# amathislab/myochallenge

Measured on AMD Instinct MI355X. Metric: env-steps/sec (Baoding, 4096 envs), higher is better.
Workload: dtype f64

## Files before the change

### include/myobatch.h

```cpp
#ifndef MYOBATCH_H
#define MYOBATCH_H

#include <stddef.h>
#include <stdint.h>

#ifdef __cplusplus
extern "C" {
#endif

#define MYO_OK 0
#define MYO_E_ARG -1
#define MYO_E_BADARG MYO_E_ARG
#define MYO_E_UNSUPPORTED -2
#define MYO_E_DEVICE -3
#define MYO_E_STATE -4

typedef struct myo_model myo_model;
typedef struct myo_batch myo_batch;

enum { MYO_F64 = 0, MYO_MIXED = 1, MYO_F32 = 1 };
enum { MYO_TASK_NONE = 0, MYO_TASK_BAODING_P1 = 1, MYO_TASK_BAODING_P2 = 2, MYO_TASK_REORIENT = 3, MYO_TASK_POSE = 4 };
enum { MYO_POSE_RESET_INIT = 0, MYO_POSE_RESET_RANDOM = 1, MYO_POSE_RESET_SDS = 2 };
enum { MYO_POSE_TARGET_GENERATE = 0, MYO_POSE_TARGET_FIXED = 1 };
enum { MYO_WHICH_HOLD = 0, MYO_WHICH_CW = 1, MYO_WHICH_CCW = 2 };
// ... 192 lines not shown
int myo_rollout_policy_input(const float* obs, int N, int O, float* obs_buf, uint16_t* x_bf16, int copies,
                             const int32_t* t_idx, void* stream);
int myo_rollout_sample(const uint16_t* mean_bf16, const uint16_t* value_bf16, const float* log_std, int N, int A,
                       uint64_t seed, uint64_t* draw_counter, const int32_t* t_idx, float* act_buf, float* val_buf,
                       float* logp_buf, float* clipped, int deterministic, void* stream);
int myo_vecnorm_step(const float* obs, const float* rew, const uint8_t* done, const uint8_t* trunc, const float* term_obs,
                     int N, int O, double* obs_mean, double* obs_var, double* obs_count, double* ret_stats,
                     double* returns, double gamma, double eps, double clip_obs, double clip_rew, int training,
                     int norm_obs, int norm_reward, float* nobs, float* starts, const int32_t* t_idx, float* rew_buf,
                     float* start_buf, float* term_buf, float* trunc_buf, double* work, void* stream);
int myo_rollout_sample_sde(const float* mean, const float* latent, const float* exploration_mat, const float* log_std, int N, int L,
                           int A, float* actions, float* clipped, float* logp, int deterministic, void* stream);

int myo_vecnorm_batch_moments(const float* obs, const float* rew, int N, int O, double* returns, double gamma, int training,
                              double* work, double* batch, void* stream);
int myo_vecnorm_finish(const float* obs, const float* rew, const uint8_t* done, const uint8_t* trunc, const float* term_obs,
                       int N, int O, double* obs_mean, double* obs_var, double* obs_count, double* ret_stats, double* returns,
                       double eps, double clip_obs, double clip_rew, int training, int norm_obs, int norm_reward, float* nobs,
                       float* starts, const int32_t* t_idx, float* rew_buf, float* start_buf, float* term_buf, float* trunc_buf,
                       const double* batch, void* stream);
int myo_rollout_advance(int32_t* t_idx, int T, uint64_t* draw_counter, void* stream);
int myo_rollout_state_snapshot(const void* h, const float* c32, int G, int N, int H, const int32_t* t_idx, int seq_len, int S,
                               void* h_snap, float* c_snap, void* stream);

int myo_lstm_cell_fwd(const void* gx, const void* gh, const void* c_prev, const float* keep_next, int R, int N, int H,
                      int is_bf16, void* out_h, void* hm_next, void* cm_next, void* c_new, void* ws, void* stream);
int myo_lstm_cell_bwd(const void* dout, const void* dhm_next, const void* dcm_next, const float* keep_next,
                      const void* c_prev, const void* c_new, const void* ws, int R, int N, int H, int is_bf16,
                      void* dgates, void* dc_prev, void* stream);

int myo_lstm_step_supported(int H);
int myo_lstm_step_fwd(const void* gx, long long gx_sg, long long gx_sr, const void* h_prev, const void* c_prev, const void* w_hh,
                      const float* keep_next, int G, int N, int H, void* out_h, long long out_sg, void* hm_next, void* cm_next,
                      void* c_new, void* ws, const float* c_prev32, float* cm_next32, void* stream);
int myo_lstm_step_bwd(const void* dout, long long dout_sg, const void* dgates_next, const void* dcm_next, const void* w_hh_t,
                      const float* keep_next, const void* c_prev, const void* c_new, const void* ws, int G, int N, int H,
                      void* dgates, void* dc_prev, void* stream);

int myo_lstm_seq_supported(int H);
int myo_lstm_seq_fwd(const void* gx, long long gx_st, long long gx_sg, long long gx_sr, void* hm, void* cm, const void* w_frag,
                     const float* keep, int G, int N, int H, int T, int row_split, void* out_h, long long out_sg, long long out_st,
                     void* c_new, void* ws, const float* c0_32, void* stream);
int myo_lstm_seq_bwd(const void* dout, long long dout_sg, long long dout_st, const void* wt_frag, const float* keep, const void* cm,
                     const void* c_new, const void* ws, int G, int N, int H, int T, int row_split, void* dgates, void* stream);

int myo_gae(const float* rew, const float* val, const float* starts, const float* last_val,
            const float* last_done, int T, int N, float gamma, float lam, float* adv, float* ret,
            void* stream);

#define MYO_HP_LR 0
#define MYO_HP_CLIP 1
#define MYO_HP_KL_LIMIT 2
#define MYO_HP_STOP 3
#define MYO_HP_APPLIED 4
#define MYO_HP_COUNT 5
#define MYO_HP_SUM_KL 6
#define MYO_HP_SUM_CLIPFRAC 7
#define MYO_HP_SUM_ENTLOSS 8
#define MYO_HP_LAST_KL 9
#define MYO_HP_LAST_PL 10
#define MYO_HP_LAST_VL 11
#define MYO_HP_WORDS 16
typedef struct myo_ppo_mlp_desc {
  const float *obs, *act, *oldlp, *adv, *ret;
  const int64_t* idx;
  int32_t B, O, A, hidden;
  const float* params;
  float* grads;
  int64_t G;
  int64_t off_W1[2], off_b1[2], off_W2[2], off_b2[2], off_Wh[2], off_bh[2], off_log_std;
  float clip, vf_coef, ent_coef;
  int32_t compute_adv_stats;
  float* adv_stats;
  float* acc;
  void* workspace;
  int64_t workspace_bytes;
  float* sqnorm_part;
  int32_t* adam_step;
  float* hp;
} myo_ppo_mlp_desc;
int myo_ppo_mlp_sqnorm_parts(int act_dim);
long long myo_ppo_mlp_workspace_bytes(int B, int obs_dim, int act_dim, int hidden, long long G);
int myo_ppo_mlp_step(const myo_ppo_mlp_desc* d, void* stream);

typedef struct myo_ppo_mlp_rollout_desc {
  const float* obs;
  int32_t N, O, A, hidden;
  const float* params;
  int64_t off_W1[2], off_b1[2], off_W2[2], off_b2[2], off_Wh[2], off_bh[2], off_log_std;
  uint64_t seed;
  uint64_t* draw_counter;
  const int32_t* t_idx;
  float *obs_buf, *act_buf, *val_buf, *logp_buf, *clipped;
  int32_t deterministic;
  void* workspace;
  int64_t workspace_bytes;
} myo_ppo_mlp_rollout_desc;
long long myo_ppo_mlp_rollout_workspace_bytes(int obs_dim, int act_dim, int hidden);
int myo_ppo_mlp_rollout_refresh(const myo_ppo_mlp_rollout_desc* d, void* stream);
int myo_ppo_mlp_rollout(const myo_ppo_mlp_rollout_desc* d, void* stream);

int myo_adam_clip_step(float* p, const float* g, float* m, float* v, int n, float lr, float b1, float b2,
                       float eps, float max_norm, float grad_scale, int* step, float* scratch, uint16_t* p_bf16,
                       void* stream);
int myo_adam_apply(float* p, const float* g, float* m, float* v, int n, float lr, float b1, float b2,
                   float eps, float max_norm, float grad_scale, const int* step, const float* scratch, int nparts,
                   uint16_t* p_bf16, void* stream);
int myo_adam_clip_step_hp(float* p, const float* g, float* m, float* v, int n, float lr, float b1, float b2,
                          float eps, float max_norm, float grad_scale, int* step, float* scratch, uint16_t* p_bf16,
                          float* hp, void* stream);
int myo_adam_apply_hp(float* p, const float* g, float* m, float* v, int n, float lr, float b1, float b2,
                      float eps, float max_norm, float grad_scale, const int* step, const float* scratch, int nparts,
                      uint16_t* p_bf16, float* hp, void* stream);

const char* myo_last_error(void);
const char* myo_version(void);

#ifdef __cplusplus
}
#endif
#endif
```

### myochallenge_amd/csrc/myo_ppo_mlp.h

```cpp
#pragma once
#ifndef MYO_EMU

typedef __attribute__((ext_vector_type(8))) __bf16 myo_bf16x8;
typedef __attribute__((ext_vector_type(4))) float myo_f32x4;

#define MLP_H 256
#define MLP_OPMAX 128
#define MLP_APM 48
#define MLP_AKP 64
#define MLP_XS (MLP_OPMAX + 8)
#define MLP_HS (MLP_H + 8)
#define MLP_DS (MLP_AKP + 8)
#define MLP_SOS 49
#define MLP_SPLITK 16

struct MlpArgs {
  const float *obs, *act, *oldlp, *adv, *ret;
  const long long* idx;
  const float *log_std, *adv_stats;
  const unsigned short *W1p, *W2, *W2T, *Whp, *WhT;
  const float* bias;
  unsigned short *XT, *H1T, *H2T, *dH1T, *dH2T, *dOT;
  float* part;
  int B, O, A, OP, NB;
  float clip, vf_coef;
  const float* hp;
};

__device__ __forceinline__ unsigned short mlp_f2bf(float x) {
  unsigned u = __float_as_uint(x);
  u += 0x7fffu + ((u >> 16) & 1u);
  return (unsigned short)(u >> 16);
}
__device__ __forceinline__ float mlp_bf2f(unsigned short h) { return __uint_as_float((unsigned)h << 16); }

struct MlpPrepArgs {
  const float* p;
  long long off_W1[2], off_b1[2], off_W2[2], off_b2[2], off_Wh[2], off_bh[2];
  int O, OP, Ah[2];
  unsigned short *W1p, *W2, *W2T, *Whp, *WhT;
  float* bias;
  const float* adv_part;
  float* adv_stats;
  int adv_nb, B;
};

#define MLP_ADV_BLOCKS 64
__global__ void __launch_bounds__(256) k_mlp_prep(MlpPrepArgs P) {
  if (P.adv_nb > 0 && blockIdx.x == gridDim.x - 1) {
    __shared__ float sp[3 * MLP_ADV_BLOCKS];
    const int t = threadIdx.x;
    if (t < 3 * P.adv_nb) sp[t] = P.adv_part[t];
    __syncthreads();
    if (t == 0) {
      float cn = 0.f, cm = 0.f, c2 = 0.f;
      for (int b = 0; b < P.adv_nb; ++b) {
        const float bn = sp[3 * b], bm = sp[3 * b + 1], b2 = sp[3 * b + 2];
        if (bn > 0.f) {
          const float tot = cn + bn, dl = bm - cm;
          cm += dl * (bn / tot);
          c2 += b2 + dl * dl * (cn * bn / tot);
          cn = tot;
        }
      }
      P.adv_stats[0] = cm; P.adv_stats[1] = sqrtf(c2 / (P.B > 1 ? P.B - 1 : 1));
    }
  }
  constexpr int H = MLP_H;
  const long long tid = (long long)blockIdx.x * blockDim.x + threadIdx.x, nth = (long long)gridDim.x * blockDim.x;
  for (int net = 0; net < 2; ++net) {
    const float* W1 = P.p + P.off_W1[net]; const float* W2 = P.p + P.off_W2[net]; const float* Wh = P.p + P.off_Wh[net];
    for (long long e = tid; e < (long long)H * P.OP; e += nth) {
      const int o = (int)(e / P.OP), i = (int)(e % P.OP);
      P.W1p[(size_t)net * H * P.OP + e] = i < P.O ? mlp_f2bf(W1[(size_t)o * P.O + i]) : (unsigned short)0;
    }
    for (long long e = tid; e < (long long)H * H; e += nth) {
      const int o = (int)(e / H), i = (int)(e % H);
      const unsigned short v = mlp_f2bf(W2[e]);
      P.W2[(size_t)net * H * H + e] = v;
      P.W2T[(size_t)net * H * H + (size_t)i * H + o] = v;
    }
    for (long long e = tid; e < (long long)MLP_APM * H; e += nth) {
      const int a = (int)(e / H), h = (int)(e % H);
      P.Whp[(size_t)net * MLP_APM * H + e] = a < P.Ah[net] ? mlp_f2bf(Wh[(size_t)a * H + h]) : (unsigned short)0;
    }
    for (long long e = tid; e < (long long)H * MLP_AKP; e += nth) {
      const int h = (int)(e / MLP_AKP), a = (int)(e % MLP_AKP);
      P.WhT[(size_t)net * H * MLP_AKP + e] = a < P.Ah[net] ? mlp_f2bf(Wh[(size_t)a * H + h]) : (unsigned short)0;
    }
    for (long long e = tid; e < H; e += nth) {
      P.bias[net * H + e] = P.p[P.off_b1[net] + e];
      P.bias[2 * H + net * H + e] = P.p[P.off_b2[net] + e];
    }
    for (long long e = tid; e < MLP_APM; e += nth) P.bias[4 * H + net * MLP_APM + e] = e < P.Ah[net] ? P.p[P.off_bh[net] + e] : 0.f;
  }
}

__global__ void __launch_bounds__(256) k_adv_moments(const float* __restrict__ adv, const long long* __restrict__ idx, int B,
                                                     float* __restrict__ part) {
  __shared__ float red[4];
  __shared__ float s_mean;
  const int t = threadIdx.x, nb = gridDim.x;
  const int chunk = (B + nb - 1) / nb, lo = blockIdx.x * chunk, hi = min(B, lo + chunk), n = max(hi - lo, 0);
  constexpr int PER = 4;
  float v[PER];
  float s = 0.f;
#pragma unroll
  for (int k = 0; k < PER; ++k) { const int i = lo + t + 256 * k; v[k] = i < hi ? adv[idx[i]] : 0.f; s += v[k]; }
  for (int i = lo + t + 256 * PER; i < hi; i += 256) s += adv[idx[i]];
  for (int off = 32; off >= 1; off >>= 1) s += __shfl_xor(s, off, 64);
  if ((t & 63) == 0) red[t >> 6] = s;
  __syncthreads();
  if (t == 0) s_mean = n ? ((red[0] + red[1]) + (red[2] + red[3])) / n : 0.f;
  __syncthreads();
  const float mean = s_mean;
  float m2 = 0.f;
#pragma unroll
  for (int k = 0; k < PER; ++k) { const float d = v[k] - mean; m2 += (lo + t + 256 * k) < hi ? d * d : 0.f; }
  for (int i = lo + t + 256 * PER; i < hi; i += 256) { const float d = adv[idx[i]] - mean; m2 += d * d; }
  for (int off = 32; off >= 1; off >>= 1) m2 += __shfl_xor(m2, off, 64);
  __syncthreads();
  if ((t & 63) == 0) red[t >> 6] = m2;
  __syncthreads();
  if (t == 0) { part[3 * blockIdx.x] = (float)n; part[3 * blockIdx.x + 1] = mean; part[3 * blockIdx.x + 2] = (red[0] + red[1]) + (red[2] + red[3]); }
}

template <int KSTEPS>
__device__ __forceinline__ void mlp_load_w(myo_bf16x8 (&bw)[8][4], const unsigned short* Wg, int w_stride, int n0, int lm, int lq) {
#pragma unroll
  for (int ks = 0; ks < KSTEPS; ++ks)
#pragma unroll
    for (int nt = 0; nt < 4; ++nt) bw[ks][nt] = *reinterpret_cast<const myo_bf16x8*>(Wg + (size_t)(n0 + 16 * nt + lm) * w_stride + 32 * ks + 8 * lq);
  __builtin_amdgcn_sched_barrier(0);
}
template <int KSTEPS, int MT>
__device__ __forceinline__ void mlp_mma_slab(myo_f32x4 (&acc)[MT][4], const unsigned short* As, int as_stride, const myo_bf16x8 (&bw)[8][4],
                                             int lm, int lq) {
#pragma unroll
  for (int mt = 0; mt < MT; ++mt)
#pragma unroll
    for (int nt = 0; nt < 4; ++nt) acc[mt][nt] = myo_f32x4{0.f, 0.f, 0.f, 0.f};
#pragma unroll
  for (int ks = 0; ks < KSTEPS; ++ks) {
#pragma unroll
    for (int m2 = 0; m2 < MT; m2 += 2) {
      myo_bf16x8 a[2];
#pragma unroll
      for (int mt = 0; mt < 2; ++mt) a[mt] = *reinterpret_cast<const myo_bf16x8*>(As + (16 * (m2 + mt) + lm) * as_stride + 32 * ks + 8 * lq);
#pragma unroll
      for (int mt = 0; mt < 2; ++mt)
#pragma unroll
        for (int nt = 0; nt < 4; ++nt) acc[m2 + mt][nt] = __builtin_amdgcn_mfma_f32_16x16x32_bf16(a[mt], bw[ks][nt], acc[m2 + mt][nt], 0, 0, 0);
    }
  }
  __builtin_amdgcn_sched_barrier(0);
}

#ifdef MLP_PROF
__device__ unsigned long long g_mlp_prof[16];
#define MLP_STAMP(k) { __syncthreads(); if (threadIdx.x == 0 && blockIdx.x == 3 && blockIdx.y == 0) g_mlp_prof[k] = wall_clock64(); }
extern "C" int myo_debug_mlp_prof(unsigned long long* out) { return (int)hipMemcpyFromSymbol(out, HIP_SYMBOL(g_mlp_prof), sizeof g_mlp_prof); }
#else
#define MLP_STAMP(k)
#endif

#ifndef MLP_BM
#define MLP_BM 32
#endif
#define MLP_FWDBWD_LDS (512 + MLP_BM * MLP_XS * 2 + MLP_BM * MLP_HS * 2 + MLP_BM * MLP_SOS * 4 + MLP_BM * MLP_DS * 2 + 128 * 4 + 192 * 4)

template <int MT>
__device__ __forceinline__ unsigned long long mlp_store_act(const myo_f32x4 (&acc)[MT][4], const float (&bb)[4], unsigned short* Hs, unsigned short* HT,
                                                            size_t B, int r0, int n0, int lm, int lq) {
  static_assert(MT * 16 <= 64, "one mask bit per accumulator element");
  unsigned long long mask = 0;
#pragma unroll
  for (int mt = 0; mt < MT; ++mt)
#pragma unroll
    for (int nt = 0; nt < 4; ++nt) {
      const int n = n0 + 16 * nt + lm, m = 16 * mt + 4 * lq;
      unsigned short h[4];
#pragma unroll
      for (int r = 0; r < 4; ++r) {
        h[r] = mlp_f2bf(fmaxf(acc[mt][nt][r] + bb[nt], 0.f)); Hs[(m + r) * MLP_HS + n] = h[r];
        mask |= (unsigned long long)(h[r] != 0) << (16 * mt + 4 * nt + r);
      }
      *reinterpret_cast<uint2*>(HT + (size_t)n * B + r0 + m) = make_uint2((unsigned)h[0] | ((unsigned)h[1] << 16), (unsigned)h[2] | ((unsigned)h[3] << 16));
    }
  return mask;
}
template <int MT, bool TO_LDS>
__device__ __forceinline__ void mlp_store_grad(const myo_f32x4 (&acc)[MT][4], unsigned long long mask, unsigned short* Hs, unsigned short* HT, size_t B,
                                               int r0, int n0, int lm, int lq) {
#pragma unroll
  for (int mt = 0; mt < MT; ++mt)
#pragma unroll
    for (int nt = 0; nt < 4; ++nt) {
      const int n = n0 + 16 * nt + lm, m = 16 * mt + 4 * lq;
      unsigned short h[4];
#pragma unroll
      for (int r = 0; r < 4; ++r) {
        const unsigned short on = (unsigned short)(-(int)((mask >> (16 * mt + 4 * nt + r)) & 1ull));
        h[r] = mlp_f2bf(acc[mt][nt][r]) & on;
        if (TO_LDS) Hs[(m + r) * MLP_HS + n] = h[r];
      }
      *reinterpret_cast<uint2*>(HT + (size_t)n * B + r0 + m) = make_uint2((unsigned)h[0] | ((unsigned)h[1] << 16), (unsigned)h[2] | ((unsigned)h[3] << 16));
    }
}

__global__ void __launch_bounds__(256, 2) k_mlp_fwdbwd(MlpArgs P) {
  constexpr int H = MLP_H, XS = MLP_XS, HS = MLP_HS, DS = MLP_DS, SOS = MLP_SOS, BM = MLP_BM, MT = BM / 16, RW = BM / 4;
  extern __shared__ __align__(16) unsigned char mlp_smem[];
  long long* s_idx = reinterpret_cast<long long*>(mlp_smem);
  unsigned short* Xs = reinterpret_cast<unsigned short*>(mlp_smem + 512);
  float* So = reinterpret_cast<float*>(mlp_smem + 512);
  unsigned short* Hs = Xs + BM * XS;
  float* Sa = reinterpret_cast<float*>(Hs + BM * HS);
  unsigned short* dOs = reinterpret_cast<unsigned short*>(Sa + BM * SOS);
  float* s_ls = reinterpret_cast<float*>(dOs + BM * DS);
  float* s_row = s_ls + 128;
  static_assert(BM * MLP_SOS * 4 <= BM * MLP_XS * 2, "the head output tile fits where X was");
  static_assert(BM == 32 || BM == 64, "wave / tile mapping below");
  const int t = threadIdx.x, w = t >> 6, lane = t & 63, lm = lane & 15, lq = lane >> 4;
  const int net = blockIdx.y, blk = blockIdx.x, r0 = blk * BM, B = P.B, O = P.O, A = P.A, OP = P.OP;
  const int n0 = 64 * w;
  MLP_STAMP(0)
  if (t < BM) s_idx[t] = P.idx[r0 + t];
  if (t < A) { const float ls = P.log_std[t]; s_ls[t] = ls; s_ls[64 + t] = __expf(-ls); }
  const float* b1 = P.bias + net * H; const float* b2 = P.bias + 2 * H + net * H; const float* bh = P.bias + 4 * H + net * MLP_APM;
  float bb1[4], bb2[4];
#pragma unroll
  for (int nt = 0; nt < 4; ++nt) { bb1[nt] = b1[n0 + 16 * nt + lm]; bb2[nt] = b2[n0 + 16 * nt + lm]; }
  myo_bf16x8 bw[8][4];
  {
    const unsigned short* W1 = P.W1p + (size_t)net * H * OP;
    if (OP == 96) mlp_load_w<3>(bw, W1, OP, n0, lm, lq);
    else if (OP == 128) mlp_load_w<4>(bw, W1, OP, n0, lm, lq);
    else if (OP == 64) mlp_load_w<2>(bw, W1, OP, n0, lm, lq);
    else mlp_load_w<1>(bw, W1, OP, n0, lm, lq);
  }
  __syncthreads();
  if (t < BM) {
    const size_t src = (size_t)s_idx[t];
// ... 303 lines not shown

__global__ void __launch_bounds__(256) k_mlp_wgrad(MlpWgradArgs P) {
  const int jid = blockIdx.x % P.njobs, split = blockIdx.x / P.njobs;
  const MlpWgradJob J = P.job[jid];
  const int t = threadIdx.x, w = t >> 6, lane = t & 63, lm = lane & 15, lq = lane >> 4;
  const int wm = w >> 1, wn = w & 1, B = P.B;
  const int mb = J.m0 + 64 * wm, nb = J.n0 + 64 * wn;
  const size_t k0 = (size_t)split * P.rows_per_split;
  myo_f32x4 acc[4][4], accb[4];
#pragma unroll
  for (int mt = 0; mt < 4; ++mt) {
    accb[mt] = myo_f32x4{0.f, 0.f, 0.f, 0.f};
#pragma unroll
    for (int nt = 0; nt < 4; ++nt) acc[mt][nt] = myo_f32x4{0.f, 0.f, 0.f, 0.f};
  }
  const bool do_bias = J.bias_off >= 0 && nb == 0;
  myo_bf16x8 ones;
#pragma unroll
  for (int j = 0; j < 8; ++j) ones[j] = (__bf16)1.0f;
  const int ksteps = P.rows_per_split / 32;
  const unsigned short* ap[4]; const unsigned short* bp[4];
#pragma unroll
  for (int q = 0; q < 4; ++q) { ap[q] = J.AT + (size_t)(mb + 16 * q + lm) * B + k0 + 8 * lq; bp[q] = J.BT + (size_t)(nb + 16 * q + lm) * B + k0 + 8 * lq; }
  myo_bf16x8 a0[4], b0[4], a1[4], b1[4];
#pragma unroll
  for (int q = 0; q < 4; ++q) { a0[q] = *reinterpret_cast<const myo_bf16x8*>(ap[q]); b0[q] = *reinterpret_cast<const myo_bf16x8*>(bp[q]); }
  for (int ks = 0; ks < ksteps; ks += 2) {
#pragma unroll
    for (int q = 0; q < 4; ++q) { a1[q] = *reinterpret_cast<const myo_bf16x8*>(ap[q] + 32 * (ks + 1)); b1[q] = *reinterpret_cast<const myo_bf16x8*>(bp[q] + 32 * (ks + 1)); }
#pragma unroll
    for (int mt = 0; mt < 4; ++mt)
#pragma unroll
      for (int nt = 0; nt < 4; ++nt) acc[mt][nt] = __builtin_amdgcn_mfma_f32_16x16x32_bf16(a0[mt], b0[nt], acc[mt][nt], 0, 0, 0);
    if (do_bias) {
#pragma unroll
      for (int mt = 0; mt < 4; ++mt) accb[mt] = __builtin_amdgcn_mfma_f32_16x16x32_bf16(a0[mt], ones, accb[mt], 0, 0, 0);
    }
    if (ks + 2 < ksteps) {
#pragma unroll
      for (int q = 0; q < 4; ++q) { a0[q] = *reinterpret_cast<const myo_bf16x8*>(ap[q] + 32 * (ks + 2)); b0[q] = *reinterpret_cast<const myo_bf16x8*>(bp[q] + 32 * (ks + 2)); }
    }
#pragma unroll
    for (int mt = 0; mt < 4; ++mt)
#pragma unroll
      for (int nt = 0; nt < 4; ++nt) acc[mt][nt] = __builtin_amdgcn_mfma_f32_16x16x32_bf16(a1[mt], b1[nt], acc[mt][nt], 0, 0, 0);
    if (do_bias) {
#pragma unroll
      for (int mt = 0; mt < 4; ++mt) accb[mt] = __builtin_amdgcn_mfma_f32_16x16x32_bf16(a1[mt], ones, accb[mt], 0, 0, 0);
    }
  }
  float* out = P.slab + (size_t)split * P.G;
#pragma unroll
  for (int mt = 0; mt < 4; ++mt)
#pragma unroll
    for (int nt = 0; nt < 4; ++nt)
#pragma unroll
      for (int r = 0; r < 4; ++r) {
        const int m = mb + 16 * mt + 4 * lq + r, n = nb + 16 * nt + lm;
        if (m < J.M && n < J.N) out[J.out_off + (size_t)m * J.ldo + n] = acc[mt][nt][r];
      }
  if (do_bias && lm == 0) {
#pragma unroll
    for (int mt = 0; mt < 4; ++mt)
#pragma unroll
      for (int r = 0; r < 4; ++r) {
        const int m = mb + 16 * mt + 4 * lq + r;
        if (m < J.M) out[J.bias_off + m] = accb[mt][r];
      }
  }
}

#define MLP_RF_BLOCKS 256
struct MlpRfArgs {
  const float* slab; float* g; long long G; int splits;
  const float* part; float* acc; int NB, A; float ent_coef;
  long long off_log_std, off_bh0, off_bh1;
  float* sq_part; int* adam_step;
  float* hp;
};
__global__ void __launch_bounds__(256) k_mlp_reduce_finish(MlpRfArgs P) {
  __shared__ float red[4];
  const int t = threadIdx.x, A = P.A;
  if ((int)blockIdx.x < MLP_RF_BLOCKS) {
    float sq = 0.f;
    for (long long e = (long long)blockIdx.x * 256 + t; e < P.G; e += (long long)MLP_RF_BLOCKS * 256) {
      float s = 0.f;
#pragma unroll 4
      for (int k = 0; k < P.splits; ++k) s += P.slab[(size_t)k * P.G + e];
      const bool theirs = (e >= P.off_log_std && e < P.off_log_std + A) || (e >= P.off_bh0 && e < P.off_bh0 + A) || e == P.off_bh1;
      if (!theirs) { P.g[e] = s; sq += s * s; }
    }
    for (int off = 32; off >= 1; off >>= 1) sq += __shfl_xor(sq, off, 64);
    if ((t & 63) == 0) red[t >> 6] = sq;
    float pl = 0.f, vl = 0.f, kl = 0.f, cf = 0.f, el = 0.f;
    if (P.hp && blockIdx.x == 0 && t < 64) {
      pl = myo_col_sum(P.part, A, P.NB, t); vl = myo_col_sum(P.part, A + 1, P.NB, t);
      kl = myo_col_sum(P.part, 2 * A + 3, P.NB, t); cf = myo_col_sum(P.part, 2 * A + 4, P.NB, t); el = myo_col_sum(P.part, 2 * A + 5, P.NB, t);
    }
    __syncthreads();
    if (t == 0) {
      P.sq_part[blockIdx.x] = (red[0] + red[1]) + (red[2] + red[3]);
      if (blockIdx.x == 0) {
        const bool stopped = P.hp ? myo_hp_record(P.hp, pl, vl, kl, cf, el) : false;
        if (!stopped) { const int done = P.adam_step[1]; P.adam_step[0] = done; P.adam_step[1] = done + 1; }
      }
    }
    return;
  }
  const int c = (int)blockIdx.x - MLP_RF_BLOCKS;
  if (t >= 64) return;
  float a = 0.f;
  for (int b = t; b < P.NB; b += 64) a += P.part[(size_t)c * P.NB + b];
  for (int off = 32; off >= 1; off >>= 1) a += __shfl_xor(a, off, 64);
  if (t == 0) {
    P.acc[c] = a;
    float w = 0.f;
    if (c < A) { w = a - P.ent_coef; P.g[P.off_log_std + c] = w; }
    else if (c >= A + 2 && c < 2 * A + 2) { w = a; P.g[P.off_bh0 + c - A - 2] = w; }
    else if (c == 2 * A + 2) { w = a; P.g[P.off_bh1] = w; }
    P.sq_part[MLP_RF_BLOCKS + c] = w * w;
  }
}

__global__ void __launch_bounds__(256) k_mlp_reduce(const float* __restrict__ slab, float* __restrict__ g, long long G, int splits) {
  const long long e = (long long)blockIdx.x * 256 + threadIdx.x;
  if (e >= G) return;
  float s = 0.f;
#pragma unroll 4
  for (int k = 0; k < splits; ++k) s += slab[(size_t)k * G + e];
  g[e] = s;
}
#endif
```

### myochallenge_amd/csrc/myobatch.hip

```cpp
#include <hip/hip_runtime.h>
#include <utility>
#include <vector>
#define MYO_BACKEND_NAME "gfx950"
#define MYO_BACKEND_DENSE_NEWTON 0
#define MYO_BACKEND_BATCH_FIELDS hipEvent_t ev0, ev1; std::vector<std::pair<hipEvent_t, hipEvent_t>> pending;
#define MYO_BACKEND_RENDER_ENVS_MAX 65535
struct DeviceGuard {
  int prev = -1; bool switched = false;
  explicit DeviceGuard(int dev) { if (hipGetDevice(&prev) == hipSuccess && prev != dev) switched = (hipSetDevice(dev) == hipSuccess); }
  ~DeviceGuard() { if (switched) (void)hipSetDevice(prev); }
};
#include "myo_host.h"

static int be_malloc(void** p, size_t n) { return (int)hipMalloc(p, n ? n : 1); }
static void be_free(void* p) { (void)hipFree(p); }
static int be_h2d(void* d, const void* h, size_t n) { return (int)hipMemcpy(d, h, n, hipMemcpyHostToDevice); }
static int be_set_device(int dev) { return (int)hipSetDevice(dev); }
static const char* be_errstr(int e) { return hipGetErrorString((hipError_t)e); }

#define MYO_MAX_DEVICES 64
struct BoundDev { const myo_batch* b = nullptr; hipStream_t last = nullptr; bool have_last = false; hipEvent_t ev = nullptr; };
static BoundDev g_bound[MYO_MAX_DEVICES];
static std::mutex g_bound_mu;
struct SlotWs { double* p = nullptr; int* map = nullptr; int users = 0; char* big = nullptr; int big_users = 0; };
// ... 531 lines not shown
                                                 const float* __restrict__ log_std, const float* __restrict__ adv_stats,
                                                 int B, int A, float clip, float vf_coef, float* __restrict__ dmean,
                                                 float* __restrict__ dvalue, float* __restrict__ acc,
                                                 unsigned short* __restrict__ dmean_h, unsigned short* __restrict__ dvalue_h,
                                                 float* __restrict__ part, const float* __restrict__ hp) {
  __shared__ float t_mean[64 * 64], t_act[64 * 64], s_ls[64], s_inv[64];
  if (hp) clip = hp[MYO_HP_CLIP];
  const int lane = threadIdx.x, r0 = blockIdx.x * 64;
  const int rows = (B - r0) < 64 ? (B - r0) : 64;
  const int n = rows * A;
  const size_t base = (size_t)r0 * A;
  const unsigned short* mean_h = reinterpret_cast<const unsigned short*>(mean);
  for (int k = lane; k < n; k += 64) {
    t_mean[k] = IN_BF16 ? __uint_as_float(((unsigned)mean_h[base + k]) << 16) : mean[base + k];
    t_act[k] = actions[base + k];
  }
  if (lane < A) { const float ls = log_std[lane]; s_ls[lane] = ls; s_inv[lane] = __expf(-ls); }
  __syncthreads();
  const int i = r0 + lane;
  const bool on = lane < rows;
  float pl_i = 0.f, vl_i = 0.f, dlogp = 0.f, dv_i = 0.f, kl_i = 0.f, cf_i = 0.f, el_i = 0.f;
  if (on) {
    float logp = 0.f, ent = 0.f;
    for (int a = 0; a < A; ++a) {
      const float z = (t_act[lane * A + a] - t_mean[lane * A + a]) * s_inv[a];
      logp += -0.5f * z * z - s_ls[a] - 0.9189385332046727f;
      ent += s_ls[a] + 1.4189385332046727f;
    }
    const float an = (adv[i] - adv_stats[0]) / (adv_stats[1] + 1e-8f);
    const float lr_i = logp - old_logp[i];
    const float ratio = __expf(lr_i);
    kl_i = ((ratio - 1.f) - lr_i) / B;
    cf_i = (fabsf(ratio - 1.f) > clip ? 1.f : 0.f) / B;
    el_i = -ent / B;
    const float s1 = an * ratio;
    const float rc = fminf(fmaxf(ratio, 1.f - clip), 1.f + clip);
    const float s2 = an * rc;
    pl_i = -fminf(s1, s2) / B;
    const bool inside = (ratio > 1.f - clip) && (ratio < 1.f + clip);
    dlogp = -(an * ratio) * ((s1 <= s2) ? 1.f : (inside ? 1.f : 0.f)) / B;
    const float val = IN_BF16 ? __uint_as_float(((unsigned)reinterpret_cast<const unsigned short*>(values)[i]) << 16) : values[i];
    const float dv = val - returns[i];
    vl_i = dv * dv / B;
    dv_i = vf_coef * 2.f / B * dv;
    dvalue[i] = dv_i;
    if (dvalue_h) dvalue_h[i] = myo_f2bf(dv_i);
  }
  if (on) {
    for (int a = 0; a < A; ++a) {
      const float inv = s_inv[a];
      const float z = (t_act[lane * A + a] - t_mean[lane * A + a]) * inv;
      t_mean[lane * A + a] = dlogp * z * inv;
      t_act[lane * A + a] = dlogp * (z * z - 1.f);
    }
  }
  __syncthreads();
  float my_ls = 0.f, my_db = 0.f;
  if (lane < A)
    for (int r = 0; r < rows; ++r) { my_ls += t_act[r * A + lane]; my_db += t_mean[r * A + lane]; }
  for (int k = lane; k < n; k += 64) {
    const float v = t_mean[k];
    dmean[base + k] = v;
    if (dmean_h) dmean_h[base + k] = myo_f2bf(v);
  }
  for (int off = 32; off >= 1; off >>= 1) {
    pl_i += __shfl_xor(pl_i, off, 64); vl_i += __shfl_xor(vl_i, off, 64); dv_i += __shfl_xor(dv_i, off, 64);
  }
  const int W = 2 * A + 3, NB = gridDim.x;
  if (lane < A) { part[(size_t)lane * NB + blockIdx.x] = my_ls; part[(size_t)(A + 2 + lane) * NB + blockIdx.x] = my_db; }
  if (lane == 0) {
    part[(size_t)A * NB + blockIdx.x] = pl_i; part[(size_t)(A + 1) * NB + blockIdx.x] = vl_i;
    part[(size_t)(2 * A + 2) * NB + blockIdx.x] = dv_i;
  }
  if (hp) {
    for (int off = 32; off >= 1; off >>= 1) {
      kl_i += __shfl_xor(kl_i, off, 64); cf_i += __shfl_xor(cf_i, off, 64); el_i += __shfl_xor(el_i, off, 64);
    }
    if (lane == 0) {
      part[(size_t)W * NB + blockIdx.x] = kl_i; part[(size_t)(W + 1) * NB + blockIdx.x] = cf_i;
      part[(size_t)(W + 2) * NB + blockIdx.x] = el_i;
    }
  }
}
__device__ __forceinline__ bool myo_hp_record(float* __restrict__ hp, float pl, float vl, float kl, float cf, float el) {
  int* hi = reinterpret_cast<int*>(hp);
  if (hi[MYO_HP_STOP]) return true;
  hp[MYO_HP_SUM_KL] += kl; hp[MYO_HP_SUM_CLIPFRAC] += cf; hp[MYO_HP_SUM_ENTLOSS] += el;
  hi[MYO_HP_COUNT] += 1;
  hp[MYO_HP_LAST_KL] = kl; hp[MYO_HP_LAST_PL] = pl; hp[MYO_HP_LAST_VL] = vl;
  const float lim = hp[MYO_HP_KL_LIMIT];
  if (lim > 0.f && kl > lim) { hi[MYO_HP_STOP] = 1; return true; }
  return false;
}
__device__ __forceinline__ float myo_col_sum(const float* __restrict__ part, int c, int NB, int lane) {
  float a = 0.f;
  for (int b = lane; b < NB; b += 64) a += part[(size_t)c * NB + b];
  for (int off = 32; off >= 1; off >>= 1) a += __shfl_xor(a, off, 64);
  return a;
}
__global__ void __launch_bounds__(64) k_colmajor_finish(const float* __restrict__ part, float* __restrict__ acc, int NB, int A,
                                                        float ent_coef, float* __restrict__ g_log_std,
                                                        float* __restrict__ g_bias_pi, float* __restrict__ g_bias_vf,
                                                        float* __restrict__ hp) {
  const int c = blockIdx.x, lane = threadIdx.x;
  if (c == 2 * A + 3) {
    const float pl = myo_col_sum(part, A, NB, lane), vl = myo_col_sum(part, A + 1, NB, lane);
    const float kl = myo_col_sum(part, c, NB, lane), cf = myo_col_sum(part, c + 1, NB, lane), el = myo_col_sum(part, c + 2, NB, lane);
    if (lane == 0) (void)myo_hp_record(hp, pl, vl, kl, cf, el);
    return;
  }
  float a = 0.f;
  for (int b = lane; b < NB; b += 64) a += part[(size_t)c * NB + b];
  for (int off = 32; off >= 1; off >>= 1) a += __shfl_xor(a, off, 64);
  if (lane == 0) {
    acc[c] = a;
    if (g_log_std && c < A) g_log_std[c] = a - ent_coef;
    if (g_bias_pi && c >= A + 2 && c < 2 * A + 2) g_bias_pi[c - A - 2] = a;
    if (g_bias_vf && c == 2 * A + 2) g_bias_vf[0] = a;
  }
}
static int ppo_loss_grad(const float* mean, const float* values, const float* actions, const float* old_logp,
                         const float* adv, const float* returns, const float* log_std, const float* adv_stats,
                         int B, int A, float clip, float vf_coef, float* dmean, float* dvalue, float* acc,
                         uint16_t* dmean_bf16, uint16_t* dvalue_bf16, float* work, int in_bf16, float ent_coef,
                         float* g_log_std, float* g_bias_pi, float* g_bias_vf, float* hp, void* stream) {
  if (!mean || !values || !actions || !old_logp || !adv || !returns || !log_std || !adv_stats || !dmean || !dvalue || !acc ||
      !work || B <= 0 || A <= 0 || A > 64)
    return fail(MYO_E_ARG, "myo_ppo_loss_grad: bad arguments");
  hipStream_t st = (hipStream_t)stream;
  const int nblk = (B + 63) / 64;
  if (in_bf16)
    hipLaunchKernelGGL(k_ppo_loss<true>, dim3(nblk), dim3(64), 0, st, mean, values, actions, old_logp, adv, returns,
                       log_std, adv_stats, B, A, clip, vf_coef, dmean, dvalue, acc, dmean_bf16, dvalue_bf16, work, (const float*)hp);
  else
    hipLaunchKernelGGL(k_ppo_loss<false>, dim3(nblk), dim3(64), 0, st, mean, values, actions, old_logp, adv, returns,
                       log_std, adv_stats, B, A, clip, vf_coef, dmean, dvalue, acc, dmean_bf16, dvalue_bf16, work, (const float*)hp);
  hipLaunchKernelGGL(k_colmajor_finish, dim3(2 * A + 3 + (hp ? 1 : 0)), dim3(64), 0, st, work, acc, nblk, A, ent_coef, g_log_std, g_bias_pi,
                     g_bias_vf, hp);
  LAUNCH_CHECK(0)
  return MYO_OK;
}
extern "C" int myo_ppo_loss_grad(const float* mean, const float* values, const float* actions, const float* old_logp,
                                 const float* adv, const float* returns, const float* log_std, const float* adv_stats,
                                 int B, int A, float clip, float vf_coef, float* dmean, float* dvalue, float* acc,
                                 uint16_t* dmean_bf16, uint16_t* dvalue_bf16, float* work, int in_bf16, float ent_coef,
                                 float* g_log_std, float* g_bias_pi, float* g_bias_vf, void* stream) {
  return ppo_loss_grad(mean, values, actions, old_logp, adv, returns, log_std, adv_stats, B, A, clip, vf_coef, dmean, dvalue, acc,
                       dmean_bf16, dvalue_bf16, work, in_bf16, ent_coef, g_log_std, g_bias_pi, g_bias_vf, nullptr, stream);
}
extern "C" int myo_ppo_loss_grad_hp(const float* mean, const float* values, const float* actions, const float* old_logp,
                                    const float* adv, const float* returns, const float* log_std, const float* adv_stats,
                                    int B, int A, float clip, float vf_coef, float* dmean, float* dvalue, float* acc,
                                    uint16_t* dmean_bf16, uint16_t* dvalue_bf16, float* work, int in_bf16, float ent_coef,
                                    float* g_log_std, float* g_bias_pi, float* g_bias_vf, float* hp, void* stream) {
  return ppo_loss_grad(mean, values, actions, old_logp, adv, returns, log_std, adv_stats, B, A, clip, vf_coef, dmean, dvalue, acc,
                       dmean_bf16, dvalue_bf16, work, in_bf16, ent_coef, g_log_std, g_bias_pi, g_bias_vf, hp, stream);
}

template <bool BF16>
__global__ void __launch_bounds__(256) k_splitk_reduce(const unsigned* __restrict__ part, float2* __restrict__ out, int splits,
                                                       int n2, int total2) {
  const int j = blockIdx.x * blockDim.x + threadIdx.x;
  if (j >= total2) return;
  const int g = j / n2, c = j - g * n2;
  float a0 = 0.f, a1 = 0.f;
  if (BF16) {
    const unsigned* src = part + (size_t)g * splits * n2 + c;
#pragma unroll 8
    for (int k = 0; k < splits; ++k) {
      const unsigned u = src[(size_t)k * n2];
      a0 += __uint_as_float(u << 16);
      a1 += __uint_as_float(u & 0xffff0000u);
    }
  } else {
    const float2* src = reinterpret_cast<const float2*>(part) + (size_t)g * splits * n2 + c;
// ... 702 lines not shown
}
template <typename E>
__global__ void __launch_bounds__(256) k_lstm_cell_bwd(const E* __restrict__ dout, const E* __restrict__ dhm_next, const E* __restrict__ dcm_next,
                                                       const float* __restrict__ keep_next, const E* __restrict__ c_prev,
                                                       const E* __restrict__ c_new, const E* __restrict__ ws, int R, int N, int H,
                                                       E* __restrict__ dgates, E* __restrict__ dc_prev) {
  const size_t idx = (size_t)blockIdx.x * blockDim.x + threadIdx.x;
  if (idx >= (size_t)R * H) return;
  const int r = (int)(idx / H), j = (int)(idx % H);
  const size_t g0 = (size_t)r * 4 * H + j;
  const float k = keep_next ? keep_next[r % N] : 1.f;
  const float dh = (dout ? myo_ld(dout, idx) : 0.f) + (dhm_next ? k * myo_ld(dhm_next, idx) : 0.f);
  const float dc_in = dcm_next ? k * myo_ld(dcm_next, idx) : 0.f;
  const float i = myo_ld(ws, g0), f = myo_ld(ws, g0 + H), g = myo_ld(ws, g0 + 2 * H), o = myo_ld(ws, g0 + 3 * H);
  const float tc = tanhf(myo_ld(c_new, idx));
  const float dct = dc_in + dh * o * (1.f - tc * tc);
  myo_st(dgates, g0, dct * g * i * (1.f - i));
  myo_st(dgates, g0 + H, dct * myo_ld(c_prev, idx) * f * (1.f - f));
  myo_st(dgates, g0 + 2 * H, dct * i * (1.f - g * g));
  myo_st(dgates, g0 + 3 * H, dh * tc * o * (1.f - o));
  myo_st(dc_prev, idx, dct * f);
}
extern "C" int myo_lstm_cell_fwd(const void* gx, const void* gh, const void* c_prev, const float* keep_next, int R, int N, int H,
                                 int is_bf16, void* out_h, void* hm_next, void* cm_next, void* c_new, void* ws, void* stream) {
  if (!gx || !gh || !c_prev || !out_h || !hm_next || !cm_next || !c_new || !ws || R <= 0 || N <= 0 || H <= 0 || R % N)
    return fail(MYO_E_ARG, "myo_lstm_cell_fwd: bad arguments");
  const unsigned nb = (unsigned)(((size_t)R * H + 255) / 256);
  if (is_bf16)
    hipLaunchKernelGGL(k_lstm_cell_fwd<unsigned short>, dim3(nb), dim3(256), 0, (hipStream_t)stream, (const unsigned short*)gx,
                       (const unsigned short*)gh, (const unsigned short*)c_prev, keep_next, R, N, H, (unsigned short*)out_h,
                       (unsigned short*)hm_next, (unsigned short*)cm_next, (unsigned short*)c_new, (unsigned short*)ws);
  else
    hipLaunchKernelGGL(k_lstm_cell_fwd<float>, dim3(nb), dim3(256), 0, (hipStream_t)stream, (const float*)gx, (const float*)gh,
                       (const float*)c_prev, keep_next, R, N, H, (float*)out_h, (float*)hm_next, (float*)cm_next, (float*)c_new,
                       (float*)ws);
  LAUNCH_CHECK(0)
  return MYO_OK;
}
extern "C" int myo_lstm_cell_bwd(const void* dout, const void* dhm_next, const void* dcm_next, const float* keep_next,
                                 const void* c_prev, const void* c_new, const void* ws, int R, int N, int H, int is_bf16,
                                 void* dgates, void* dc_prev, void* stream) {
  if (!c_prev || !c_new || !ws || !dgates || !dc_prev || R <= 0 || N <= 0 || H <= 0 || R % N)
    return fail(MYO_E_ARG, "myo_lstm_cell_bwd: bad arguments");
  const unsigned nb = (unsigned)(((size_t)R * H + 255) / 256);
  if (is_bf16)
    hipLaunchKernelGGL(k_lstm_cell_bwd<unsigned short>, dim3(nb), dim3(256), 0, (hipStream_t)stream, (const unsigned short*)dout,
                       (const unsigned short*)dhm_next, (const unsigned short*)dcm_next, keep_next, (const unsigned short*)c_prev,
                       (const unsigned short*)c_new, (const unsigned short*)ws, R, N, H, (unsigned short*)dgates,
                       (unsigned short*)dc_prev);
  else
    hipLaunchKernelGGL(k_lstm_cell_bwd<float>, dim3(nb), dim3(256), 0, (hipStream_t)stream, (const float*)dout, (const float*)dhm_next,
                       (const float*)dcm_next, keep_next, (const float*)c_prev, (const float*)c_new, (const float*)ws, R, N, H,
                       (float*)dgates, (float*)dc_prev);
  LAUNCH_CHECK(0)
  return MYO_OK;
}

__global__ void k_gae(const float* __restrict__ rew, const float* __restrict__ val, const float* __restrict__ starts,
                      const float* __restrict__ last_val, const float* __restrict__ last_done, int T, int N, float gamma,
                      float lam, float* __restrict__ adv, float* __restrict__ ret) {
  const int e = blockIdx.x * blockDim.x + threadIdx.x;
  if (e >= N) return;
  float last = 0.f, nextv = last_val[e], nonterm = 1.f - last_done[e];
  for (int t = T - 1; t >= 0; --t) {
    const size_t i = (size_t)t * N + e;
    const float v = val[i];
    const float delta = rew[i] + gamma * nextv * nonterm - v;
    last = delta + gamma * lam * nonterm * last;
    adv[i] = last;
    ret[i] = last + v;
    nextv = v;
    nonterm = 1.f - starts[i];
  }
}
extern "C" int myo_gae(const float* rew, const float* val, const float* starts, const float* last_val, const float* last_done,
                       int T, int N, float gamma, float lam, float* adv, float* ret, void* stream) {
  if (!rew || !val || !starts || !last_val || !last_done || !adv || !ret || T <= 0 || N <= 0) return fail(MYO_E_ARG, "myo_gae: bad arguments");
  hipLaunchKernelGGL(k_gae, dim3((N + 255) / 256), dim3(256), 0, (hipStream_t)stream, rew, val, starts, last_val, last_done, T, N,
                     gamma, lam, adv, ret);
  LAUNCH_CHECK(0)
  return MYO_OK;
}

#define MYO_SQN_BLOCKS 64
__global__ void __launch_bounds__(256) k_grad_sqnorm(const float* __restrict__ g, int n, float gs, float* __restrict__ part,
                                                     int* __restrict__ step, const float* __restrict__ hp) {
  float acc = 0.f;
  for (int i = blockIdx.x * 256 + threadIdx.x; i < n; i += MYO_SQN_BLOCKS * 256) { const float x = g[i] * gs; acc += x * x; }
  for (int off = 32; off >= 1; off >>= 1) acc += __shfl_xor(acc, off, 64);
  __shared__ float red[4];
  if ((threadIdx.x & 63) == 0) red[threadIdx.x >> 6] = acc;
  __syncthreads();
  if (threadIdx.x == 0) {
    part[blockIdx.x] = (red[0] + red[1]) + (red[2] + red[3]);
    if (blockIdx.x == 0 && !(hp && reinterpret_cast<const int*>(hp)[MYO_HP_STOP])) { const int done = step[1]; step[0] = done; step[1] = done + 1; }
  }
}
__global__ void __launch_bounds__(256) k_adam(float* __restrict__ p, const float* __restrict__ g, float* __restrict__ m,
                                              float* __restrict__ v, int n, float lr, float b1, float b2, float eps,
                                              float max_norm, float gs, const int* __restrict__ step,
                                              const float* __restrict__ part, unsigned short* __restrict__ p_bf16, int nparts,
                                              float* __restrict__ hp) {
  if (hp) {
    if (reinterpret_cast<const int*>(hp)[MYO_HP_STOP]) return;
    lr = hp[MYO_HP_LR];
  }
  __shared__ float sq_red[256];
  {
    float a = 0.f;
    for (int k = threadIdx.x; k < nparts; k += 256) a += part[k];
    sq_red[threadIdx.x] = a;
    __syncthreads();
    for (int w = 128; w >= 1; w >>= 1) { if ((int)threadIdx.x < w) sq_red[threadIdx.x] += sq_red[threadIdx.x + w]; __syncthreads(); }
  }
  const float sq = sq_red[0];
  const int t = step[1];
  const float norm = sqrtf(sq);
  const float clip = (max_norm > 0.f) ? fminf(1.f, max_norm / (norm + 1e-6f)) : 1.f;
  const float bc1 = 1.f - powf(b1, (float)t), bc2 = 1.f - powf(b2, (float)t);
  const float step_size = lr / bc1, inv_sqrt_bc2 = rsqrtf(bc2);
  for (int i = blockIdx.x * blockDim.x + threadIdx.x; i < n; i += gridDim.x * blockDim.x) {
    const float gi = g[i] * gs * clip;
    const float mi = b1 * m[i] + (1.f - b1) * gi;
    const float vi = b2 * v[i] + (1.f - b2) * gi * gi;
    m[i] = mi; v[i] = vi;
    const float pn = p[i] - step_size * mi / (sqrtf(vi) * inv_sqrt_bc2 + eps);
    p[i] = pn;
    if (p_bf16) p_bf16[i] = myo_f2bf(pn);
  }
  if (hp && blockIdx.x == 0 && threadIdx.x == 0) reinterpret_cast<int*>(hp)[MYO_HP_APPLIED] += 1;
}
static int adam_clip_step(float* p, const float* g, float* m, float* v, int n, float lr, float b1, float b2,
                          float eps, float max_norm, float grad_scale, int* step, float* scratch, uint16_t* p_bf16,
                          float* hp, void* stream) {
  if (!p || !g || !m || !v || !step || !scratch || n <= 0) return fail(MYO_E_ARG, "myo_adam_clip_step: bad arguments");
  hipStream_t st = (hipStream_t)stream;
  const int blocks = (n + 255) / 256 < 1024 ? (n + 255) / 256 : 1024;
  hipLaunchKernelGGL(k_grad_sqnorm, dim3(MYO_SQN_BLOCKS), dim3(256), 0, st, g, n, grad_scale, scratch, step, (const float*)hp);
  hipLaunchKernelGGL(k_adam, dim3(blocks), dim3(256), 0, st, p, g, m, v, n, lr, b1, b2, eps, max_norm, grad_scale, step, scratch,
                     (unsigned short*)p_bf16, MYO_SQN_BLOCKS, hp);
  LAUNCH_CHECK(0)
  return MYO_OK;
}
extern "C" int myo_adam_clip_step(float* p, const float* g, float* m, float* v, int n, float lr, float b1, float b2,
                                  float eps, float max_norm, float grad_scale, int* step, float* scratch, uint16_t* p_bf16,
                                  void* stream) {
  return adam_clip_step(p, g, m, v, n, lr, b1, b2, eps, max_norm, grad_scale, step, scratch, p_bf16, nullptr, stream);
}
extern "C" int myo_adam_clip_step_hp(float* p, const float* g, float* m, float* v, int n, float lr, float b1, float b2,
                                     float eps, float max_norm, float grad_scale, int* step, float* scratch, uint16_t* p_bf16,
                                     float* hp, void* stream) {
  return adam_clip_step(p, g, m, v, n, lr, b1, b2, eps, max_norm, grad_scale, step, scratch, p_bf16, hp, stream);
}
static int adam_apply(float* p, const float* g, float* m, float* v, int n, float lr, float b1, float b2,
                      float eps, float max_norm, float grad_scale, const int* step, const float* scratch, int nparts,
                      uint16_t* p_bf16, float* hp, void* stream) {
  if (!p || !g || !m || !v || !step || !scratch || n <= 0 || nparts <= 0) return fail(MYO_E_ARG, "myo_adam_apply: bad arguments");
  const int blocks = (n + 255) / 256 < 1024 ? (n + 255) / 256 : 1024;
  hipLaunchKernelGGL(k_adam, dim3(blocks), dim3(256), 0, (hipStream_t)stream, p, g, m, v, n, lr, b1, b2, eps, max_norm, grad_scale, step, scratch,
                     (unsigned short*)p_bf16, nparts, hp);
  LAUNCH_CHECK(0)
  return MYO_OK;
}
extern "C" int myo_adam_apply(float* p, const float* g, float* m, float* v, int n, float lr, float b1, float b2,
                              float eps, float max_norm, float grad_scale, const int* step, const float* scratch, int nparts,
                              uint16_t* p_bf16, void* stream) {
  return adam_apply(p, g, m, v, n, lr, b1, b2, eps, max_norm, grad_scale, step, scratch, nparts, p_bf16, nullptr, stream);
}
extern "C" int myo_adam_apply_hp(float* p, const float* g, float* m, float* v, int n, float lr, float b1, float b2,
                                 float eps, float max_norm, float grad_scale, const int* step, const float* scratch, int nparts,
                                 uint16_t* p_bf16, float* hp, void* stream) {
  return adam_apply(p, g, m, v, n, lr, b1, b2, eps, max_norm, grad_scale, step, scratch, nparts, p_bf16, hp, stream);
}

#include "myo_ppo_mlp.h"
struct MlpWs { unsigned short *W1p, *W2, *W2T, *Whp, *WhT; float* bias; unsigned short *XT, *H1T, *H2T, *dH1T, *dH2T, *dOT; float *part, *slab, *advpart; size_t bytes; };
static MlpWs mlp_carve(unsigned char* base, int B, int OP, int A, long long G) {
  MlpWs w;
  size_t o = 0;
  auto take = [&](size_t n) { unsigned char* p = base ? base + o : nullptr; o += (n + 255) / 256 * 256; return p; };
  const size_t H = MLP_H;
  w.W1p = (unsigned short*)take(2 * H * OP * 2); w.W2 = (unsigned short*)take(2 * H * H * 2); w.W2T = (unsigned short*)take(2 * H * H * 2);
  w.Whp = (unsigned short*)take(2 * MLP_APM * H * 2); w.WhT = (unsigned short*)take(2 * H * MLP_AKP * 2);
  w.bias = (float*)take((4 * H + 2 * MLP_APM) * 4);
  w.XT = (unsigned short*)take((size_t)128 * B * 2);
  w.H1T = (unsigned short*)take(2 * H * (size_t)B * 2); w.H2T = (unsigned short*)take(2 * H * (size_t)B * 2);
  w.dH1T = (unsigned short*)take(2 * H * (size_t)B * 2); w.dH2T = (unsigned short*)take(2 * H * (size_t)B * 2);
  w.dOT = (unsigned short*)take((size_t)256 * B * 2);
  w.part = (float*)take((size_t)(2 * A + 6) * (B / MLP_BM) * 4);
  w.slab = (float*)take((size_t)MLP_SPLITK * G * 4);
  w.advpart = (float*)take(3 * MLP_ADV_BLOCKS * 4);
  w.bytes = o;
  return w;
}
static int mlp_shape_ok(int B, int O, int A, int hidden) {
  return hidden == MLP_H && O >= 1 && O <= MLP_OPMAX && A >= 1 && A <= MLP_APM && B >= 64 * MLP_SPLITK && B % (64 * MLP_SPLITK) == 0;
}
extern "C" long long myo_ppo_mlp_workspace_bytes(int B, int obs_dim, int act_dim, int hidden, long long G) {
  if (!mlp_shape_ok(B, obs_dim, act_dim, hidden) || G <= 0) return -1;
  return (long long)mlp_carve(nullptr, B, (obs_dim + 31) / 32 * 32, act_dim, G).bytes;
}
extern "C" int myo_ppo_mlp_sqnorm_parts(int act_dim) {
  return MLP_RF_BLOCKS + 2 * act_dim + 3;
}
extern "C" int myo_ppo_mlp_step(const myo_ppo_mlp_desc* d, void* stream) {
  if (!d || !d->obs || !d->act || !d->oldlp || !d->adv || !d->ret || !d->idx || !d->params || !d->grads || !d->adv_stats || !d->acc ||
      !d->workspace)
    return fail(MYO_E_ARG, "myo_ppo_mlp_step: null argument");
  const int B = d->B, O = d->O, A = d->A, OP = (O + 31) / 32 * 32;
  if (!mlp_shape_ok(B, O, A, d->hidden)) return fail(MYO_E_UNSUPPORTED, "myo_ppo_mlp_step: needs hidden = %d, obs <= %d, act <= %d, batch a multiple of %d", MLP_H, MLP_OPMAX, MLP_APM, 64 * MLP_SPLITK);
  const MlpWs w = mlp_carve((unsigned char*)d->workspace, B, OP, A, d->G);
  if ((long long)w.bytes > d->workspace_bytes) return fail(MYO_E_ARG, "myo_ppo_mlp_step: workspace too small (%zu bytes needed)", w.bytes);
  hipStream_t st = (hipStream_t)stream;
  static bool lds_set = false;
  if (!lds_set) {
    if (hipFuncSetAttribute((const void*)k_mlp_fwdbwd, hipFuncAttributeMaxDynamicSharedMemorySize, MLP_FWDBWD_LDS) != hipSuccess)
      return fail(MYO_E_DEVICE, "myo_ppo_mlp_step: cannot reserve %d bytes of LDS", (int)MLP_FWDBWD_LDS);
    lds_set = true;
  }
  if (d->compute_adv_stats) hipLaunchKernelGGL(k_adv_moments, dim3(MLP_ADV_BLOCKS), dim3(256), 0, st, d->adv, (const long long*)d->idx, B, w.advpart);
  MlpPrepArgs pp;
  pp.p = d->params; pp.O = O; pp.OP = OP; pp.Ah[0] = A; pp.Ah[1] = 1;
  for (int k = 0; k < 2; ++k) {
    pp.off_W1[k] = d->off_W1[k]; pp.off_b1[k] = d->off_b1[k]; pp.off_W2[k] = d->off_W2[k]; pp.off_b2[k] = d->off_b2[k];
    pp.off_Wh[k] = d->off_Wh[k]; pp.off_bh[k] = d->off_bh[k];
  }
  pp.adv_part = w.advpart; pp.adv_stats = d->adv_stats; pp.adv_nb = d->compute_adv_stats ? MLP_ADV_BLOCKS : 0; pp.B = B;
  pp.W1p = w.W1p; pp.W2 = w.W2; pp.W2T = w.W2T; pp.Whp = w.Whp; pp.WhT = w.WhT; pp.bias = w.bias;
  hipLaunchKernelGGL(k_mlp_prep, dim3(256), dim3(256), 0, st, pp);
  MlpArgs a;
  a.obs = d->obs; a.act = d->act; a.oldlp = d->oldlp; a.adv = d->adv; a.ret = d->ret; a.idx = (const long long*)d->idx;
  a.log_std = d->params + d->off_log_std; a.adv_stats = d->adv_stats;
  a.W1p = w.W1p; a.W2 = w.W2; a.W2T = w.W2T; a.Whp = w.Whp; a.WhT = w.WhT; a.bias = w.bias;
  a.XT = w.XT; a.H1T = w.H1T; a.H2T = w.H2T; a.dH1T = w.dH1T; a.dH2T = w.dH2T; a.dOT = w.dOT; a.part = w.part;
  a.B = B; a.O = O; a.A = A; a.OP = OP; a.NB = B / MLP_BM; a.clip = d->clip; a.vf_coef = d->vf_coef; a.hp = d->hp;
  hipLaunchKernelGGL(k_mlp_fwdbwd, dim3(B / MLP_BM, 2), dim3(256), MLP_FWDBWD_LDS, st, a);
  MlpWgradArgs g;
  g.njobs = 0; g.B = B; g.rows_per_split = B / MLP_SPLITK; g.G = d->G; g.slab = w.slab;
  const size_t HB = (size_t)MLP_H * B;
  for (int net = 0; net < 2; ++net) {
    for (int m0 = 0; m0 < MLP_H; m0 += 128) {
      for (int n0 = 0; n0 < MLP_H; n0 += 128)
        g.job[g.njobs++] = MlpWgradJob{w.dH2T + net * HB, w.H1T + net * HB, MLP_H, MLP_H, MLP_H, m0, n0, d->off_W2[net], n0 == 0 ? d->off_b2[net] : -1};
      g.job[g.njobs++] = MlpWgradJob{w.dH1T + net * HB, w.XT, MLP_H, O, O, m0, 0, d->off_W1[net], d->off_b1[net]};
    }
    for (int n0 = 0; n0 < MLP_H; n0 += 128)
      g.job[g.njobs++] = MlpWgradJob{w.dOT + (size_t)net * 128 * B, w.H2T + net * HB, net == 0 ? A : 1, MLP_H, MLP_H, 0, n0, d->off_Wh[net], -1};
  }
  hipLaunchKernelGGL(k_mlp_wgrad, dim3(g.njobs * MLP_SPLITK), dim3(256), 0, st, g);
  if (d->sqnorm_part && d->adam_step) {
    MlpRfArgs rf;
    rf.slab = w.slab; rf.g = d->grads; rf.G = d->G; rf.splits = MLP_SPLITK; rf.part = w.part; rf.acc = d->acc; rf.NB = B / MLP_BM; rf.A = A;
    rf.ent_coef = d->ent_coef; rf.off_log_std = d->off_log_std; rf.off_bh0 = d->off_bh[0]; rf.off_bh1 = d->off_bh[1];
    rf.sq_part = d->sqnorm_part; rf.adam_step = d->adam_step; rf.hp = d->hp;
    hipLaunchKernelGGL(k_mlp_reduce_finish, dim3(MLP_RF_BLOCKS + 2 * A + 3), dim3(256), 0, st, rf);
  } else {
    hipLaunchKernelGGL(k_mlp_reduce, dim3((unsigned)((d->G + 255) / 256)), dim3(256), 0, st, (const float*)w.slab, d->grads, d->G, MLP_SPLITK);
    hipLaunchKernelGGL(k_colmajor_finish, dim3(2 * A + 3 + (d->hp ? 1 : 0)), dim3(64), 0, st, (const float*)w.part, d->acc, B / MLP_BM, A, d->ent_coef,
                       d->grads + d->off_log_std, d->grads + d->off_bh[0], d->grads + d->off_bh[1], d->hp);
  }
  LAUNCH_CHECK(0)
  return MYO_OK;
}

struct MlpImg { unsigned short *W1p, *W2, *W2T, *Whp, *WhT; float* bias; size_t bytes; };
static MlpImg mlp_carve_images(unsigned char* base, int OP) {
  MlpImg w;
  size_t o = 0;
  auto take = [&](size_t n) { unsigned char* p = base ? base + o : nullptr; o += (n + 255) / 256 * 256; return p; };
  const size_t H = MLP_H;
  w.W1p = (unsigned short*)take(2 * H * OP * 2); w.W2 = (unsigned short*)take(2 * H * H * 2); w.W2T = (unsigned short*)take(2 * H * H * 2);
  w.Whp = (unsigned short*)take(2 * MLP_APM * H * 2); w.WhT = (unsigned short*)take(2 * H * MLP_AKP * 2);
  w.bias = (float*)take((4 * H + 2 * MLP_APM) * 4);
  w.bytes = o;
  return w;
}
static int mlp_rollout_ok(const myo_ppo_mlp_rollout_desc* d) {
  return d->hidden == MLP_H && d->O >= 1 && d->O <= MLP_OPMAX && d->A >= 1 && d->A <= MLP_APM && d->N >= MLP_BM && d->N % MLP_BM == 0;
}
extern "C" long long myo_ppo_mlp_rollout_workspace_bytes(int obs_dim, int act_dim, int hidden) {
  if (hidden != MLP_H || obs_dim < 1 || obs_dim > MLP_OPMAX || act_dim < 1 || act_dim > MLP_APM) return -1;
  return (long long)mlp_carve_images(nullptr, (obs_dim + 31) / 32 * 32).bytes;
}
extern "C" int myo_ppo_mlp_rollout_refresh(const myo_ppo_mlp_rollout_desc* d, void* stream) {
  if (!d || !d->params || !d->workspace) return fail(MYO_E_ARG, "myo_ppo_mlp_rollout_refresh: null argument");
  if (!mlp_rollout_ok(d)) return fail(MYO_E_UNSUPPORTED, "myo_ppo_mlp_rollout: needs hidden = %d, obs <= %d, act <= %d, envs a multiple of %d", MLP_H, MLP_OPMAX, MLP_APM, MLP_BM);
  const int OP = (d->O + 31) / 32 * 32;
  const MlpImg w = mlp_carve_images((unsigned char*)d->workspace, OP);
  if ((long long)w.bytes > d->workspace_bytes) return fail(MYO_E_ARG, "myo_ppo_mlp_rollout_refresh: workspace too small (%zu bytes needed)", w.bytes);
  MlpPrepArgs pp;
  pp.p = d->params; pp.O = d->O; pp.OP = OP; pp.Ah[0] = d->A; pp.Ah[1] = 1;
  for (int k = 0; k < 2; ++k) {
    pp.off_W1[k] = d->off_W1[k]; pp.off_b1[k] = d->off_b1[k]; pp.off_W2[k] = d->off_W2[k]; pp.off_b2[k] = d->off_b2[k];
    pp.off_Wh[k] = d->off_Wh[k]; pp.off_bh[k] = d->off_bh[k];
  }
  pp.adv_part = nullptr; pp.adv_stats = nullptr; pp.adv_nb = 0; pp.B = 0;
  pp.W1p = w.W1p; pp.W2 = w.W2; pp.W2T = w.W2T; pp.Whp = w.Whp; pp.WhT = w.WhT; pp.bias = w.bias;
  hipLaunchKernelGGL(k_mlp_prep, dim3(256), dim3(256), 0, (hipStream_t)stream, pp);
  LAUNCH_CHECK(0)
  return MYO_OK;
}
extern "C" int myo_ppo_mlp_rollout(const myo_ppo_mlp_rollout_desc* d, void* stream) {
  if (!d || !d->obs || !d->params || !d->draw_counter || !d->t_idx || !d->act_buf || !d->val_buf || !d->logp_buf || !d->clipped || !d->workspace)
    return fail(MYO_E_ARG, "myo_ppo_mlp_rollout: null argument");
  if (!mlp_rollout_ok(d)) return fail(MYO_E_UNSUPPORTED, "myo_ppo_mlp_rollout: needs hidden = %d, obs <= %d, act <= %d, envs a multiple of %d", MLP_H, MLP_OPMAX, MLP_APM, MLP_BM);
  const int OP = (d->O + 31) / 32 * 32;
  const MlpImg w = mlp_carve_images((unsigned char*)d->workspace, OP);
  if ((long long)w.bytes > d->workspace_bytes) return fail(MYO_E_ARG, "myo_ppo_mlp_rollout: workspace too small (%zu bytes needed)", w.bytes);
  MlpPolicyArgs a;
  a.obs = d->obs; a.log_std = d->params + d->off_log_std; a.W1p = w.W1p; a.W2 = w.W2; a.Whp = w.Whp; a.bias = w.bias;
  a.obs_buf = d->obs_buf; a.act_buf = d->act_buf; a.val_buf = d->val_buf; a.logp_buf = d->logp_buf; a.clipped = d->clipped;
  a.t_idx = d->t_idx; a.draw_counter = (unsigned long long*)d->draw_counter; a.seed = d->seed;
  a.N = d->N; a.O = d->O; a.A = d->A; a.OP = OP; a.deterministic = d->deterministic;
  hipLaunchKernelGGL(k_mlp_policy, dim3(d->N / MLP_BM, 2), dim3(256), MLP_POLICY_LDS, (hipStream_t)stream, a);
  LAUNCH_CHECK(0)
  return MYO_OK;
}

#include "myo_lstm_step.h"
extern "C" int myo_lstm_step_supported(int H) { return (H == 32 || H == 64 || H == 128 || H == 256) ? 1 : 0; }
extern "C" int myo_lstm_step_fwd(const void* gx, long long gx_sg, long long gx_sr, const void* h_prev, const void* c_prev, const void* w_hh,
                                 const float* keep_next, int G, int N, int H, void* out_h, long long out_sg, void* hm_next, void* cm_next,
                                 void* c_new, void* ws, const float* c_prev32, float* cm_next32, void* stream) {
  if (!gx || !h_prev || (!c_prev && !c_prev32) || !w_hh || !out_h || !hm_next || (!cm_next && !cm_next32) || G <= 0 || N <= 0 || H <= 0 || (gx_sg & 3) || (gx_sr & 3) || (out_sg & 3))
    return fail(MYO_E_ARG, "myo_lstm_step_fwd: bad arguments");
  if (!myo_lstm_step_supported(H)) return fail(MYO_E_UNSUPPORTED, "myo_lstm_step_fwd: hidden size %d (32, 64, 128 or 256)", H);
  typedef const unsigned short* cu;
  typedef unsigned short* mu;
#define MYO_LSTM_FWD(HH)                                                                                                              \
  lstm_step_fwd_launch<HH>((cu)gx, gx_sg, gx_sr, (cu)h_prev, (cu)c_prev, (cu)w_hh, keep_next, G, N, (mu)out_h, out_sg, (mu)hm_next,   \
                           (mu)cm_next, (mu)c_new, (mu)ws, c_prev32, cm_next32, (hipStream_t)stream)
  switch (H) {
    case 32: MYO_LSTM_FWD(32); break;
    case 64: MYO_LSTM_FWD(64); break;
    case 128: MYO_LSTM_FWD(128); break;
    default: MYO_LSTM_FWD(256); break;
  }
#undef MYO_LSTM_FWD
  LAUNCH_CHECK(0)
  return MYO_OK;
}
extern "C" int myo_lstm_step_bwd(const void* dout, long long dout_sg, const void* dgates_next, const void* dcm_next, const void* w_hh_t,
                                 const float* keep_next, const void* c_prev, const void* c_new, const void* ws, int G, int N, int H,
// ... 55 lines not shown
```

### myochallenge_amd/native.py

```python
from __future__ import annotations

import ctypes as C
import os
from typing import Optional

import numpy as np

_HERE = os.path.dirname(os.path.abspath(__file__))
LIB_PATH = os.path.join(_HERE, "libmyobatch.so")

MYO_F64, MYO_MIXED = 0, 1
MYO_F32 = MYO_MIXED
TASK_NONE, TASK_BAODING_P1, TASK_BAODING_P2, TASK_REORIENT, TASK_POSE = 0, 1, 2, 3, 4
POSE_RESET_INIT, POSE_RESET_RANDOM, POSE_RESET_SDS = 0, 1, 2
POSE_TARGET_GENERATE, POSE_TARGET_FIXED = 0, 1
CHOICE_FIXED, CHOICE_CW, CHOICE_CCW, CHOICE_RANDOM = 0, 1, 2, 3
MUSCLE_NONE, MUSCLE_FATIGUE, MUSCLE_REAFFERENTATION = 0, 1, 2
N_RWD = 8
RWD_KEYS = ("pos_dist_1", "pos_dist_2", "act_reg", "alive", "sparse", "solved", "done", "dense")


ROT_CHOICE_MAX, OBJG_MAX, POSE_NQ_MAX = 4, 20, 38


# ... 114 lines not shown
        vp, i32, u64, dbl = C.c_void_p, C.c_int, C.c_uint64, C.c_double
        L.myo_last_error.restype = C.c_char_p
        L.myo_version.restype = C.c_char_p
        L.myo_model_from_blob.argtypes = [vp, C.c_size_t, C.POINTER(vp)]
        L.myo_model_load_mjb.argtypes = [C.c_char_p, i32, i32, C.POINTER(vp)]
        L.myo_model_destroy.argtypes = [vp]
        L.myo_model_size.argtypes = [vp, C.c_char_p]
        L.myo_batch_create.argtypes = [vp, C.POINTER(TaskCfg), i32, i32, u64, i32, C.POINTER(vp)]
        L.myo_batch_destroy.argtypes = [vp]
        L.myo_batch_num_envs.argtypes = [vp]
        L.myo_batch_set_step_generation.argtypes = [vp, C.c_uint32]
        L.myo_batch_health.argtypes = [vp, C.POINTER(i32)]
        L.myo_debug_wave_slots.argtypes = [C.c_int, C.c_int, C.c_int, C.POINTER(i32)]
        L.myo_batch_obs_dim.argtypes = [vp]
        L.myo_batch_lds_bytes.argtypes = [vp]
        L.myo_batch_reset.argtypes = [vp, vp, vp, vp]
        L.myo_batch_step.argtypes = [vp] * 10
        L.myo_batch_step_inner.argtypes = [vp] * 6
        L.myo_batch_step_inner_idx.argtypes = [vp, vp, i32, vp, vp, vp, vp]
        L.myo_batch_copy_envs.argtypes = [vp, vp, vp, vp, i32, vp]
        L.myo_batch_physics_step.argtypes = [vp, vp, i32, vp]
        L.myo_batch_get_state.argtypes = [vp] * 6
        L.myo_batch_set_state.argtypes = [vp] * 6
        L.myo_batch_set_task.argtypes = [vp] * 5
        L.myo_batch_warmstart.argtypes = [vp] * 4
        L.myo_batch_set_bad_state_buffer.argtypes = [vp, vp]
        L.myo_batch_get_task.argtypes = [vp] * 5
        L.myo_batch_bind_constants.argtypes = [vp, vp]
        L.myo_batch_tune_wrap_order.argtypes = [vp, vp]
        L.myo_batch_set_object_group.argtypes = [vp, i32, i32]
        L.myo_batch_object_friction.argtypes = [vp, vp, vp, vp]
        L.myo_batch_fatigue.argtypes = [vp, vp, vp, vp]
        L.myo_batch_forward_dump.argtypes = [vp, vp, vp, vp]
        L.myo_batch_dump_size.argtypes = [vp]
        L.myo_batch_dump_offset.argtypes = [vp, C.c_char_p]
        L.myo_batch_kernel_ms.argtypes = [vp]
        L.myo_batch_kernel_ms.restype = dbl
        L.myo_batch_enable_timing.argtypes = [vp, i32]
        L.myo_model_default_camera.argtypes = [vp, C.POINTER(RenderCamera)]
        L.myo_batch_geom_poses.argtypes = [vp, vp, i32, vp, vp]
        L.myo_batch_tendon_paths.argtypes = [vp, vp, i32, vp, vp]
        L.myo_batch_render.argtypes = [vp, vp, i32, C.POINTER(RenderCamera), i32, i32, i32, i32, vp, vp, vp, vp]
        L.myo_batch_contact_items.argtypes = [vp, vp, i32, vp, vp]
        L.myo_batch_set_render_style.argtypes = [vp, C.POINTER(RenderStyle)]
        L.myo_batch_get_render_style.argtypes = [vp, C.POINTER(RenderStyle)]
        L.myo_batch_contact_capacity.argtypes = [vp]
        L.myo_batch_sense.argtypes = [vp, C.POINTER(SenseOut), vp]
        L.myo_batch_data.argtypes = [vp, vp, C.POINTER(DataOut), vp]
        if b"MYO_EMU" in L.myo_version():
            return
        L.myo_ppo_loss_grad.argtypes = [vp] * 8 + [i32, i32, C.c_float, C.c_float, vp, vp, vp, vp, vp, vp, i32, C.c_float, vp, vp, vp, vp]
        L.myo_ppo_loss_grad_hp.argtypes = L.myo_ppo_loss_grad.argtypes[:-1] + [vp, vp]
        L.myo_ppo_gather.argtypes = [vp] * 6 + [i32, i32, i32, vp, i32] + [vp] * 7
        L.myo_ppo_gather_seq.argtypes = [vp] * 9 + [i32] * 8 + [vp, i32] + [vp] * 11
        L.myo_rollout_state_snapshot.argtypes = [vp, vp, i32, i32, i32, vp, i32, i32, vp, vp, vp]
        L.myo_bias_relu_bf16.argtypes = [vp, vp, i32, i32, i32, vp]
        L.myo_splitk_reduce.argtypes = [vp, i32, vp, i32, i32, i32, vp]
        L.myo_splitk_reduce2.argtypes = [vp, i32, vp, i32, i32, i32, vp, i32, vp, i32, i32, i32, vp]
        L.myo_relu_bwd_colsum_bf16.argtypes = [vp, vp, i32, i32, vp, vp]
        L.myo_rollout_policy_input.argtypes = [vp, i32, i32, vp, vp, i32, vp, vp]
        L.myo_rollout_sample.argtypes = [vp, vp, vp, i32, i32, u64, vp, vp, vp, vp, vp, vp, i32, vp]
        L.myo_vecnorm_step.argtypes = [vp] * 5 + [i32, i32] + [vp] * 5 + [dbl] * 4 + [i32] * 3 + [vp] * 9
        L.myo_rollout_advance.argtypes = [vp, i32, vp, vp]
        L.myo_rollout_sample_sde.argtypes = [vp] * 4 + [i32] * 3 + [vp] * 3 + [i32, vp]
        L.myo_vecnorm_batch_moments.argtypes = [vp, vp, i32, i32, vp, dbl, i32, vp, vp, vp]
        L.myo_vecnorm_finish.argtypes = [vp] * 5 + [i32, i32] + [vp] * 5 + [dbl] * 3 + [i32] * 3 + [vp] * 9
        L.myo_gae.argtypes = [vp] * 5 + [i32, i32, C.c_float, C.c_float, vp, vp, vp]
        L.myo_lstm_cell_fwd.argtypes = [vp] * 4 + [i32] * 4 + [vp] * 6
        L.myo_lstm_cell_bwd.argtypes = [vp] * 7 + [i32] * 4 + [vp] * 3
        L.myo_lstm_step_supported.argtypes = [i32]
        L.myo_lstm_step_fwd.argtypes = [vp, C.c_longlong, C.c_longlong] + [vp] * 4 + [i32] * 3 + [vp, C.c_longlong] + [vp] * 7
        L.myo_lstm_step_bwd.argtypes = [vp, C.c_longlong] + [vp] * 7 + [i32] * 3 + [vp] * 3
        L.myo_lstm_seq_supported.argtypes = [i32]
        L.myo_lstm_seq_fwd.argtypes = [vp] + [C.c_longlong] * 3 + [vp] * 4 + [i32] * 5 + [vp, C.c_longlong, C.c_longlong] + [vp] * 4
        L.myo_lstm_seq_bwd.argtypes = [vp, C.c_longlong, C.c_longlong] + [vp] * 5 + [i32] * 5 + [vp] * 2
        L.myo_adam_clip_step.argtypes = [vp] * 4 + [i32] + [C.c_float] * 6 + [vp, vp, vp, vp]
        L.myo_adam_apply.argtypes = [vp] * 4 + [i32] + [C.c_float] * 6 + [vp, vp, i32, vp, vp]
        L.myo_adam_clip_step_hp.argtypes = L.myo_adam_clip_step.argtypes[:-1] + [vp, vp]
        L.myo_adam_apply_hp.argtypes = L.myo_adam_apply.argtypes[:-1] + [vp, vp]
        L.myo_ppo_mlp_workspace_bytes.restype = C.c_longlong
        L.myo_ppo_mlp_workspace_bytes.argtypes = [i32, i32, i32, i32, C.c_longlong]
        L.myo_ppo_mlp_step.argtypes = [C.POINTER(PpoMlpDesc), vp]
        L.myo_ppo_mlp_sqnorm_parts.argtypes = [i32]
        L.myo_ppo_mlp_rollout_workspace_bytes.restype = C.c_longlong
        L.myo_ppo_mlp_rollout_workspace_bytes.argtypes = [i32, i32, i32]
        L.myo_ppo_mlp_rollout_refresh.argtypes = [C.POINTER(PpoMlpRolloutDesc), vp]
        L.myo_ppo_mlp_rollout.argtypes = [C.POINTER(PpoMlpRolloutDesc), vp]

    def check(self, rc: int):
        if rc != 0:
            raise MyoError(f"libmyobatch error {rc}: {self.L.myo_last_error().decode()}")

    @property
    def version(self) -> str:
        return self.L.myo_version().decode()

    @property
    def build_id(self) -> str:
        v = self.version
        return v.rsplit(" build ", 1)[1] if " build " in v else "unknown"

    @property
    def is_emulation(self) -> bool:
        return "MYO_EMU" in self.version


_LIB: Optional[NativeLib] = None


def load(path: Optional[str] = None) -> NativeLib:
    global _LIB
    if path is not None:
        return NativeLib(path)
    if _LIB is None:
        _LIB = NativeLib(LIB_PATH)
    return _LIB


EXPORTED_SYMBOLS = [
    "myo_model_from_blob", "myo_model_load_mjb", "myo_model_destroy", "myo_model_size", "myo_batch_create",
    "myo_batch_destroy", "myo_batch_set_step_generation", "myo_batch_health", "myo_debug_wave_slots", "myo_batch_num_envs", "myo_batch_obs_dim", "myo_batch_lds_bytes",
    "myo_batch_reset", "myo_batch_step", "myo_batch_step_inner", "myo_batch_step_inner_idx", "myo_batch_copy_envs", "myo_batch_physics_step", "myo_batch_get_state",
    "myo_batch_set_state", "myo_batch_warmstart", "myo_batch_set_bad_state_buffer", "myo_batch_set_task", "myo_batch_get_task", "myo_batch_set_object_group", "myo_batch_object_friction", "myo_batch_bind_constants", "myo_batch_tune_wrap_order", "myo_batch_forward_dump",
    "myo_batch_dump_size", "myo_batch_dump_offset", "myo_batch_kernel_ms",
    "myo_batch_enable_timing", "myo_ppo_loss_grad", "myo_ppo_gather", "myo_ppo_gather_seq", "myo_rollout_state_snapshot", "myo_bias_relu_bf16", "myo_rollout_policy_input", "myo_rollout_sample",
    "myo_vecnorm_step", "myo_rollout_sample_sde", "myo_vecnorm_batch_moments", "myo_vecnorm_finish", "myo_rollout_advance", "myo_gae", "myo_lstm_cell_fwd", "myo_lstm_cell_bwd", "myo_lstm_step_supported", "myo_lstm_step_fwd", "myo_lstm_step_bwd", "myo_lstm_seq_supported", "myo_lstm_seq_fwd", "myo_lstm_seq_bwd", "myo_splitk_reduce", "myo_splitk_reduce2", "myo_relu_bwd_colsum_bf16", "myo_adam_clip_step", "myo_ppo_mlp_workspace_bytes", "myo_ppo_mlp_step", "myo_ppo_mlp_sqnorm_parts", "myo_adam_apply", "myo_ppo_mlp_rollout_workspace_bytes", "myo_ppo_mlp_rollout_refresh", "myo_ppo_mlp_rollout", "myo_ppo_loss_grad_hp", "myo_adam_clip_step_hp", "myo_adam_apply_hp", "myo_last_error", "myo_version",
    "myo_model_default_camera", "myo_batch_geom_poses", "myo_batch_tendon_paths", "myo_batch_render",
    "myo_batch_contact_capacity", "myo_batch_sense", "myo_batch_data",
    "myo_batch_contact_items", "myo_batch_set_render_style", "myo_batch_get_render_style",
    "myo_batch_fatigue",
]

ENV_PATH_SYMBOLS = [
    "myo_batch_bind_constants", "myo_batch_copy_envs", "myo_batch_create", "myo_batch_destroy", "myo_batch_dump_offset", "myo_batch_dump_size",
    "myo_batch_enable_timing", "myo_batch_forward_dump", "myo_batch_get_state", "myo_batch_get_task", "myo_batch_health", "myo_batch_kernel_ms",
    "myo_batch_lds_bytes", "myo_batch_num_envs", "myo_batch_object_friction", "myo_batch_obs_dim", "myo_batch_physics_step", "myo_batch_reset",
    "myo_batch_set_bad_state_buffer", "myo_batch_set_object_group", "myo_batch_set_state", "myo_batch_set_step_generation", "myo_batch_set_task",
    "myo_batch_step", "myo_batch_step_inner", "myo_batch_step_inner_idx", "myo_batch_tune_wrap_order", "myo_batch_warmstart", "myo_debug_wave_slots",
    "myo_last_error", "myo_model_destroy", "myo_model_from_blob", "myo_model_load_mjb", "myo_model_size", "myo_version",
    "myo_model_default_camera", "myo_batch_geom_poses", "myo_batch_tendon_paths", "myo_batch_render",
    "myo_batch_contact_capacity", "myo_batch_sense", "myo_batch_data",
    "myo_batch_contact_items", "myo_batch_set_render_style", "myo_batch_get_render_style",
    "myo_batch_fatigue",
]


class Model:

    def __init__(self, compiled, lib: Optional[NativeLib] = None):
        self.lib = lib or load()
        self.compiled = compiled
        blob = compiled.to_blob()
        self._buf = C.create_string_buffer(blob, len(blob))
        h = C.c_void_p()
        self.lib.check(self.lib.L.myo_model_from_blob(self._buf, len(blob), C.byref(h)))
        self.h = h

    @classmethod
    def from_mjb(cls, path: str, lib: Optional[NativeLib] = None, integrator: Optional[int] = None, unsupported_contacts: str = "error",
                 allow_other_solver: bool = False):
        self = cls.__new__(cls)
        self.lib, self.compiled, self._buf = lib or load(), None, None
        h = C.c_void_p()
        self.lib.check(self.lib.L.myo_model_load_mjb(os.fsencode(path), -1 if integrator is None else int(integrator),
                                                     {"error": 0, "drop": 1}[unsupported_contacts] | (2 if allow_other_solver else 0), C.byref(h)))
        self.h = h
        return self

    def size(self, name: str) -> int:
        return self.lib.L.myo_model_size(self.h, name.encode())

    def default_camera(self) -> dict:
        c = RenderCamera()
        self.lib.check(self.lib.L.myo_model_default_camera(self.h, C.byref(c)))
        return {"lookat": tuple(c.lookat), "distance": c.distance, "azimuth": c.azimuth, "elevation": c.elevation, "fovy": c.fovy}

    def __del__(self):
        if getattr(self, "h", None):
            self.lib.L.myo_model_destroy(self.h)
            self.h = None


def _ptr(x):
    if x is None:
        return None
    if isinstance(x, int):
        return x
    if isinstance(x, np.ndarray):
        assert x.flags["C_CONTIGUOUS"]
        return x.ctypes.data
    return x.data_ptr()


class Batch:

    def __init__(self, model: Model, cfg: Optional[TaskCfg], n_envs: int, device: int = 0, seed: int = 0,
                 dtype: int = MYO_F32):
        self.lib, self.model = model.lib, model
        h = C.c_void_p()
        self.lib.check(self.lib.L.myo_batch_create(model.h, C.byref(cfg) if cfg is not None else None,
                                                   n_envs, device, seed, dtype, C.byref(h)))
        self.h = h
        self.n = n_envs
        self.dtype = dtype
        self.obs_dim = self.lib.L.myo_batch_obs_dim(h)

    def reset(self, mask=None, obs=None, stream=None):
        self.lib.check(self.lib.L.myo_batch_reset(self.h, _ptr(mask), _ptr(obs), stream))

    def step(self, act, obs, rew, done, trunc=None, term_obs=None, comps=None, ep_info=None, stream=None):
        self.lib.check(self.lib.L.myo_batch_step(self.h, _ptr(act), _ptr(obs), _ptr(rew), _ptr(done), _ptr(trunc),
                                                 _ptr(term_obs), _ptr(comps), _ptr(ep_info), stream))

# ... 153 lines not shown
```

### myochallenge_amd/rl/fused_mlp.py

```python
from __future__ import annotations

import ctypes as C
import math
from typing import List, Tuple

import torch


def _layers(seq) -> List[torch.nn.Linear]:
    return [m for m in seq if isinstance(m, torch.nn.Linear)]


def _nets(policy):
    return {"pi": _layers(policy.mlp_extractor.policy_net) + [policy.action_net],
            "vf": _layers(policy.mlp_extractor.value_net) + [policy.value_net]}


def _splitk_wgrad(dy: torch.Tensor, x: torch.Tensor, split: int) -> Tuple[torch.Tensor, torch.Tensor]:
    B = x.shape[0]
    if split > 1 and B % split == 0:
        gw = torch.bmm(dy.view(split, B // split, -1).transpose(1, 2), x.view(split, B // split, -1)).sum(0, dtype=torch.float32)
    else:
        gw = (dy.t() @ x).float()
    return gw, dy.sum(0, dtype=torch.float32)
# ... 34 lines not shown
    dmean = dlogp.unsqueeze(-1) * z * inv_std
    dlogstd = (dlogp.unsqueeze(-1) * (z * z - 1)).sum(0) - ent_coef
    dvalue = (vf_coef * 2.0 / B) * (values - returns)

    def put(p, g):
        if p.grad is None:
            p.grad = g.clone()
        else:
            p.grad.copy_(g)
    put(policy.log_std, dlogstd)
    for name, dout in (("pi", dmean), ("vf", dvalue.unsqueeze(-1))):
        layers, saved = nets[name], acts[name]
        dy = dout.to(cd)
        for li in reversed(range(len(layers))):
            lin = layers[li]
            gw, gb = _splitk_wgrad(dy, saved[li], split_k)
            put(lin.weight, gw)
            put(lin.bias, gb)
            if li > 0:
                dy = (dy @ lin.weight.to(cd)) * (saved[li] > 0).to(cd)
    return pl, vl


def _colsum(x):
    xf = x.float()
    ones = torch.ones((*xf.shape[:-2], 1, xf.shape[-2]), device=x.device)
    return torch.matmul(ones, xf).squeeze(-2)


def flatten_parameters(policy, pad: int = 64):
    if getattr(policy, "_flat", None) is not None:
        return policy._flat
    params = list(policy.parameters())
    pi, vf = _layers(policy.mlp_extractor.policy_net), _layers(policy.mlp_extractor.value_net)
    lead = []
    if len(pi) == len(vf) and all(a.weight.shape == b.weight.shape for a, b in zip(pi, vf)):
        for a, b in zip(pi, vf):
            lead += [a.weight, b.weight, a.bias, b.bias]
    la, lc = getattr(policy, "lstm_actor", None), getattr(policy, "lstm_critic", None)
    if policy.recurrent and lc is not None and la.hidden_size == lc.hidden_size:
        for key in ("weight_ih_l0", "weight_hh_l0", "bias_ih_l0", "bias_hh_l0"):
            lead += [getattr(la, key), getattr(lc, key)]
    ids = {id(p) for p in lead}
    params = lead + [p for p in params if id(p) not in ids]
    dev = params[0].device
    slots, n = [], 0
    for p in params:
        slots.append((n, p.numel()))
        n += (p.numel() + pad - 1) // pad * pad
    pflat, gflat = torch.zeros(n, device=dev), torch.zeros(n, device=dev)
    for p, (off, k) in zip(params, slots):
        pflat[off:off + k].copy_(p.data.reshape(-1))
        p.data = pflat[off:off + k].view(p.shape)
        p.grad = gflat[off:off + k].view(p.shape)
    policy._flat = {"p": pflat, "g": gflat, "slots": slots, "params": params}
    return policy._flat


def hp_record_torch(hp, pl, vl, kl, cf, el):
    from ..native import HP_COUNT, HP_KL_LIMIT, HP_LAST_KL, HP_LAST_VL, HP_STOP, HP_SUM_ENTLOSS, HP_SUM_KL
    hi = hp.view(torch.int32)
    live = hi[HP_STOP] == 0
    zero = torch.zeros((), device=hp.device)
    hp[HP_SUM_KL:HP_SUM_ENTLOSS + 1].add_(torch.where(live, torch.stack([kl, cf, el]).float(), zero))
    hi[HP_COUNT].add_(live.to(torch.int32))
    last = hp[HP_LAST_KL:HP_LAST_VL + 1]
    last.copy_(torch.where(live, torch.stack([kl, pl, vl]).float(), last))
    lim = hp[HP_KL_LIMIT]
    hi[HP_STOP].bitwise_or_((live & (lim > 0) & (kl > lim)).to(torch.int32))


class FlatAdam:

    def __init__(self, flat, lib, lr, max_norm, betas=(0.9, 0.999), eps=1e-5):
        self.flat, self.lib = flat, lib
        self.lr, self.max_norm, self.betas, self.eps = float(lr), float(max_norm), betas, float(eps)
        dev = flat["p"].device
        self.m, self.v = torch.zeros_like(flat["p"]), torch.zeros_like(flat["p"])
        self._step = torch.zeros(2, dtype=torch.int32, device=dev)
        self.sq = torch.zeros(512, device=dev)
        self.presummed = 0
        self.shadow = None
        self.hp = None

    @property
    def step_count(self):
        return self._step[1]

    def set_step_count(self, step: float) -> None:
        self._step.fill_(int(step))

    def step(self, grad_scale: float = 1.0):
        f = self.flat
        stream = torch.cuda.current_stream(f["p"].device).cuda_stream
        p = lambda t: C.c_void_p(t.data_ptr())
        if self.hp is not None:
            sh = p(self.shadow) if self.shadow is not None else None
            if self.presummed > 0:
                self.lib.check(self.lib.L.myo_adam_apply_hp(
                    p(f["p"]), p(f["g"]), p(self.m), p(self.v), f["p"].numel(), self.lr, self.betas[0], self.betas[1],
                    self.eps, self.max_norm, float(grad_scale), p(self._step), p(self.sq), int(self.presummed), sh, p(self.hp),
                    C.c_void_p(stream)))
            else:
                self.lib.check(self.lib.L.myo_adam_clip_step_hp(
                    p(f["p"]), p(f["g"]), p(self.m), p(self.v), f["p"].numel(), self.lr, self.betas[0], self.betas[1],
                    self.eps, self.max_norm, float(grad_scale), p(self._step), p(self.sq), sh, p(self.hp), C.c_void_p(stream)))
            return
        if self.presummed > 0:
            self.lib.check(self.lib.L.myo_adam_apply(
                p(f["p"]), p(f["g"]), p(self.m), p(self.v), f["p"].numel(), self.lr, self.betas[0], self.betas[1],
                self.eps, self.max_norm, float(grad_scale), p(self._step), p(self.sq), int(self.presummed),
                p(self.shadow) if self.shadow is not None else None, C.c_void_p(stream)))
            return
        self.lib.check(self.lib.L.myo_adam_clip_step(
            p(f["p"]), p(f["g"]), p(self.m), p(self.v), f["p"].numel(), self.lr, self.betas[0], self.betas[1],
            self.eps, self.max_norm, float(grad_scale), p(self._step), p(self.sq),
            p(self.shadow) if self.shadow is not None else None, C.c_void_p(stream)))

    def snapshot(self):
        return [t.clone() for t in (self.flat["p"], self.m, self.v, self._step)]

    def restore(self, snap):
        for t, s in zip((self.flat["p"], self.m, self.v, self._step), snap):
            t.copy_(s)
        if self.shadow is not None:
            self.shadow.copy_(self.flat["p"])


class FusedPPOStep:

    def __init__(self, policy, lib, clip_range, ent_coef, vf_coef, split_k=64):
        self.policy, self.lib = policy, lib
        self.clip, self.ent, self.vf, self.split = float(clip_range), float(ent_coef), float(vf_coef), split_k
        self.adam_syncs_shadow = False
        self.nets = _nets(policy)
        dev = policy.log_std.device
        self.master, self.half = [], []
        self.wb = {}
        flat = getattr(policy, "_flat", None)
        if flat is not None:
            hflat = torch.empty_like(flat["p"], dtype=torch.bfloat16)
            self.master, self.half = [flat["p"]], [hflat]
            for p, (off, k) in zip(flat["params"], flat["slots"]):
                self.wb[id(p)] = hflat[off:off + k].view(p.shape)
        else:
            for name, layers in self.nets.items():
                for lin in layers:
                    for p in (lin.weight, lin.bias):
                        if p.grad is None:
                            p.grad = torch.zeros_like(p)
                        h = torch.empty_like(p, dtype=torch.bfloat16)
                        self.master.append(p.data)
                        self.half.append(h)
                        self.wb[id(p)] = h
        if policy.log_std.grad is None:
            policy.log_std.grad = torch.zeros_like(policy.log_std)
        A = policy.act_dim
        self.merged = None
        if flat is not None:
            self.merged = self._stacked_views(flat, hflat)
        self.acc = torch.zeros(2 * A + 4, device=dev)
        self.stats = torch.zeros(2, device=dev)
        self.external_adv_stats = False
        self.A = A
        self._work = {}
        self._mfma = {}
        self.use_mfma_step = True
        self.adam = None
        self.hp = None

    def _mfma_desc(self, B, obs_all, act_all, oldlp_all, adv_all, ret_all, idx):
        from .. import native
        flat = getattr(self.policy, "_flat", None)
        if not self.use_mfma_step or flat is None or self.merged is None or len(self.merged) != 2 or self.policy.recurrent:
            return None
        pi, vf = self.nets["pi"], self.nets["vf"]
        O = obs_all.shape[1]
        hid = pi[0].weight.shape[0]
        shapes_ok = all(tuple(l.weight.shape) == s for l, s in ((pi[0], (hid, O)), (vf[0], (hid, O)), (pi[1], (hid, hid)), (vf[1], (hid, hid)),
                                                               (pi[2], (self.A, hid)), (vf[2], (1, hid))))
        if not shapes_ok or self.policy.log_std.dim() != 1 or obs_all.dtype != torch.float32:
            return None
        G = flat["p"].numel()
        key = (B, O, self.A, hid, G)
        hit = self._mfma.get(key)
        if hit is not None:
            d = hit[0]
            if d is not None:
                d.obs, d.act, d.oldlp, d.adv, d.ret, d.idx = (t.data_ptr() for t in (obs_all, act_all, oldlp_all, adv_all, ret_all, idx))
                d.hp = self.hp.data_ptr() if self.hp is not None else None
            return d
        nbytes = self.lib.L.myo_ppo_mlp_workspace_bytes(B, O, self.A, hid, G)
        if nbytes <= 0:
            self._mfma[key] = (None, None)
            return None
        ws = torch.zeros(nbytes, dtype=torch.uint8, device=obs_all.device)
        slot = {id(p): sl[0] for p, sl in zip(flat["params"], flat["slots"])}
        d = native.PpoMlpDesc()
        d.obs, d.act, d.oldlp, d.adv, d.ret, d.idx = (t.data_ptr() for t in (obs_all, act_all, oldlp_all, adv_all, ret_all, idx))
        d.B, d.O, d.A, d.hidden = B, O, self.A, hid
        d.params, d.grads, d.G = flat["p"].data_ptr(), flat["g"].data_ptr(), G
        for k, (a, b) in enumerate(zip(pi, vf)):
            for net, lin in enumerate((a, b)):
                wname, bname = (("off_W1", "off_b1"), ("off_W2", "off_b2"), ("off_Wh", "off_bh"))[k]
                getattr(d, wname)[net] = slot[id(lin.weight)]
                getattr(d, bname)[net] = slot[id(lin.bias)]
        d.off_log_std = slot[id(self.policy.log_std)]
        d.clip, d.vf_coef, d.ent_coef = self.clip, self.vf, self.ent
        d.adv_stats, d.acc = self.stats.data_ptr(), self.acc.data_ptr()
        d.workspace, d.workspace_bytes = ws.data_ptr(), nbytes
        d.hp = self.hp.data_ptr() if self.hp is not None else None
        if self.adam is not None and self.lib.L.myo_ppo_mlp_sqnorm_parts(self.A) <= self.adam.sq.numel():
            d.sqnorm_part, d.adam_step = self.adam.sq.data_ptr(), self.adam._step.data_ptr()
        self._mfma[key] = (d, ws)
        return d

    def rollout_desc(self, obs, seed, draw, t_idx, obs_buf, act_buf, val_buf, logp_buf, clipped):
        from .. import native
        flat = getattr(self.policy, "_flat", None)
        if not self.use_mfma_step or flat is None or self.merged is None or len(self.merged) != 2 or self.policy.recurrent:
            return None
        pi, vf = self.nets["pi"], self.nets["vf"]
        N, O = obs.shape
        hid = pi[0].weight.shape[0]
        shapes_ok = all(tuple(l.weight.shape) == s for l, s in ((pi[0], (hid, O)), (vf[0], (hid, O)), (pi[1], (hid, hid)), (vf[1], (hid, hid)),
                                                               (pi[2], (self.A, hid)), (vf[2], (1, hid))))
        if not shapes_ok or self.policy.log_std.dim() != 1 or obs.dtype != torch.float32 or N % 32:
            return None
        nbytes = self.lib.L.myo_ppo_mlp_rollout_workspace_bytes(O, self.A, hid)
        if nbytes <= 0:
            return None
        ws = torch.zeros(nbytes, dtype=torch.uint8, device=obs.device)
        slot = {id(p): sl[0] for p, sl in zip(flat["params"], flat["slots"])}
        d = native.PpoMlpRolloutDesc()
        d.obs, d.N, d.O, d.A, d.hidden, d.params = obs.data_ptr(), N, O, self.A, hid, flat["p"].data_ptr()
        for k, (a, b) in enumerate(zip(pi, vf)):
            for net, lin in enumerate((a, b)):
                wname, bname = (("off_W1", "off_b1"), ("off_W2", "off_b2"), ("off_Wh", "off_bh"))[k]
                getattr(d, wname)[net] = slot[id(lin.weight)]
                getattr(d, bname)[net] = slot[id(lin.bias)]
        d.off_log_std = slot[id(self.policy.log_std)]
        d.seed, d.draw_counter, d.t_idx = seed, draw.data_ptr(), t_idx.data_ptr()
        d.obs_buf, d.act_buf, d.val_buf, d.logp_buf, d.clipped = (t.data_ptr() for t in (obs_buf, act_buf, val_buf, logp_buf, clipped))
        d.deterministic, d.workspace, d.workspace_bytes = 0, ws.data_ptr(), nbytes
        self._rollout = (d, ws)
        self.refresh_rollout_images()
        return d

    def refresh_rollout_images(self):
        r = getattr(self, "_rollout", None)
        if r is not None:
            stream = torch.cuda.current_stream(self.acc.device).cuda_stream
            self.lib.check(self.lib.L.myo_ppo_mlp_rollout_refresh(C.byref(r[0]), C.c_void_p(stream)))

    def rollout_policy(self, d):
        stream = torch.cuda.current_stream(self.acc.device).cuda_stream
        self.lib.check(self.lib.L.myo_ppo_mlp_rollout(C.byref(d), C.c_void_p(stream)))

    def _mfma_step(self, d):
        d.compute_adv_stats = 0 if self.external_adv_stats else 1
        stream = torch.cuda.current_stream(self.acc.device).cuda_stream
        self.lib.check(self.lib.L.myo_ppo_mlp_step(C.byref(d), C.c_void_p(stream)))
        if self.adam is not None:
            self.adam.presummed = self.lib.L.myo_ppo_mlp_sqnorm_parts(self.A) if d.sqnorm_part else 0
        return self.acc[self.A], self.acc[self.A + 1]

    def _workbuf(self, key, n):
        w = self._work.get((key, n))
        if w is None:
            w = self._work[(key, n)] = torch.zeros(n, device=self.acc.device)
        return w

    def _stacked_views(self, flat, hflat):
        pi, vf = self.nets["pi"][:-1], self.nets["vf"][:-1]
        if len(pi) != len(vf) or (not pi and not self.policy.recurrent):
            return None
        slot = {id(p): sl for p, sl in zip(flat["params"], flat["slots"])}
        out = []
        for a, b in zip(pi, vf):
            lay = {}
            for key, pa, pb in (("w", a.weight, b.weight), ("b", a.bias, b.bias)):
                (oa, k), (ob, kb) = slot[id(pa)], slot[id(pb)]
                if pa.shape != pb.shape or ob != oa + k:
                    return None
                shape = (2,) + tuple(pa.shape)
                lay[key + "h"] = hflat[oa:oa + 2 * k].view(shape)
                lay[key + "g"] = flat["g"][oa:oa + 2 * k].view(shape)
            out.append(lay)
        return out

    def _reduce(self, part, out, groups, splits):
        n = out.numel() // groups
        stream = torch.cuda.current_stream(out.device).cuda_stream
        self.lib.check(self.lib.L.myo_splitk_reduce(C.c_void_p(part.data_ptr()), int(part.dtype == torch.bfloat16),
                                                    C.c_void_p(out.data_ptr()), groups, splits, n, C.c_void_p(stream)))

    def _reduce2(self, part_a, out_a, groups_a, splits_a, part_b, out_b, groups_b, splits_b):
        stream = torch.cuda.current_stream(out_a.device).cuda_stream
        self.lib.check(self.lib.L.myo_splitk_reduce2(
            C.c_void_p(part_a.data_ptr()), int(part_a.dtype == torch.bfloat16), C.c_void_p(out_a.data_ptr()), groups_a, splits_a,
            out_a.numel() // groups_a, C.c_void_p(part_b.data_ptr()), int(part_b.dtype == torch.bfloat16),
            C.c_void_p(out_b.data_ptr()), groups_b, splits_b, out_b.numel() // groups_b, C.c_void_p(stream)))

    def _relu_bwd_partial(self, dh, act):
        G, B, H = dh.shape
        if not (B % 32 == 0 and H % 16 == 0 and 256 % (H // 2) == 0):
            return None
        partial = torch.empty((G * B // 32, H), device=dh.device)
        stream = torch.cuda.current_stream(dh.device).cuda_stream
        self.lib.check(self.lib.L.myo_relu_bwd_colsum_bf16(C.c_void_p(dh.data_ptr()), C.c_void_p(act.data_ptr()), G * B, H,
                                                           C.c_void_p(partial.data_ptr()), C.c_void_p(stream)))
        return partial

    def _relu_bwd_bias(self, dh, act, bias_grad):
        G, B, H = dh.shape
        if B % 32 == 0 and H % 16 == 0 and 256 % (H // 2) == 0:
            partial = torch.empty((G * B // 32, H), device=dh.device)
            stream = torch.cuda.current_stream(dh.device).cuda_stream
            self.lib.check(self.lib.L.myo_relu_bwd_colsum_bf16(C.c_void_p(dh.data_ptr()), C.c_void_p(act.data_ptr()), G * B, H,
                                                               C.c_void_p(partial.data_ptr()), C.c_void_p(stream)))
            self._reduce(partial, bias_grad, G, B // 32)
            return dh
        dh = torch.ops.aten.threshold_backward(dh, act, 0)
        bias_grad.copy_(_colsum(dh))
        return dh

    def _loss_kernel(self, mean, values, actions, old_logp, adv, returns, dmean_h=None, dvalue_h=None, direct=None):
        pol = self.policy
        B, A = mean.shape[0], self.A
        in_bf16 = int(mean.dtype == torch.bfloat16)
        assert values.dtype == mean.dtype
        d = direct or (None, None, None)
        dev = mean.device
        dmean, dvalue = torch.empty((B, A), device=dev), torch.empty(B, device=dev)
        work = self._workbuf("loss", ((B + 63) // 64) * (2 * A + 6))
        stream = torch.cuda.current_stream(dev).cuda_stream
        p = lambda t: C.c_void_p(t.data_ptr()) if t is not None else None
        if self.hp is not None:
            self.lib.check(self.lib.L.myo_ppo_loss_grad_hp(
                p(mean), p(values), p(actions), p(old_logp), p(adv), p(returns), p(pol.log_std.data), p(self.stats),
                B, A, self.clip, self.vf, p(dmean), p(dvalue), p(self.acc), p(dmean_h), p(dvalue_h), p(work), in_bf16, self.ent,
                p(d[0]), p(d[1]), p(d[2]), p(self.hp), C.c_void_p(stream)))
            return dmean, dvalue
        self.lib.check(self.lib.L.myo_ppo_loss_grad(
            p(mean), p(values), p(actions), p(old_logp), p(adv), p(returns), p(pol.log_std.data), p(self.stats),
# ... 190 lines not shown
```

### myochallenge_amd/rl/ppo.py

```python
from __future__ import annotations

import os
import time
import warnings
from collections import deque
from dataclasses import dataclass, field
from typing import Callable, Dict, Optional

import torch
import torch.distributed as dist

from .. import native
from ..native import (HP_APPLIED, HP_CLIP, HP_COUNT, HP_LAST_KL, HP_LAST_PL, HP_LAST_VL, HP_STOP, HP_SUM_ENTLOSS, HP_SUM_KL,
                      HP_WORDS)
from .fused_lstm import FusedRecurrentPPOStep
from .fused_mlp import FlatAdam, FusedPPOStep, flatten_parameters, hp_record_torch
from .policy import ActorCriticPolicy


@dataclass
class PPOConfig:
    n_steps: int = 128
    batch_size: int = 4096
    n_epochs: int = 10
# ... 28 lines not shown
        if self.lr_schedule is not None:
            self.learning_rate = float(self.lr_schedule(1.0))
        if self.clip_range_schedule is not None:
            self.clip_range = float(self.clip_range_schedule(1.0))


def compute_gae(rewards, values, episode_starts, last_values, last_dones, gamma, lam):
    T = rewards.shape[0]
    if rewards.is_cuda and rewards.dtype == torch.float32:
        import ctypes as C
        lib = native.load()
        adv, ret = torch.empty_like(rewards), torch.empty_like(rewards)
        p = lambda t: C.c_void_p(t.contiguous().data_ptr())
        lv, ld = last_values.float().contiguous(), last_dones.float().contiguous()
        lib.check(lib.L.myo_gae(p(rewards), p(values), p(episode_starts), p(lv), p(ld), T, rewards.shape[1],
                                float(gamma), float(lam), p(adv), p(ret),
                                C.c_void_p(torch.cuda.current_stream(rewards.device).cuda_stream)))
        return adv, ret
    adv = torch.zeros_like(rewards)
    last = torch.zeros_like(last_values)
    for t in reversed(range(T)):
        if t == T - 1:
            nonterm, nextv = 1.0 - last_dones, last_values
        else:
            nonterm, nextv = 1.0 - episode_starts[t + 1], values[t + 1]
        delta = rewards[t] + gamma * nextv * nonterm - values[t]
        last = delta + gamma * lam * nonterm * last
        adv[t] = last
    return adv, adv + values


class PPO:
    def __init__(self, env, policy: ActorCriticPolicy, cfg: PPOConfig = PPOConfig(), seed: int = 0):
        self.env, self.policy, self.cfg = env, policy, cfg
        self.device = env.device
        self.policy.to(self.device)
        on_gpu = self.device.type == "cuda"
        if cfg.target_kl is not None and (cfg.graph_allreduce or os.environ.get("MYO_GRAPH_ALLREDUCE") == "1"):
            raise ValueError("target_kl needs the host between gradient and optimizer step on N > 1 ranks (the all-reduced approx_kl "
                             "decides): it cannot be combined with graph_allreduce")
        if cfg.seq_len is not None:
            if not policy.recurrent:
                raise ValueError("seq_len cuts the sequences of a recurrent policy: this policy has no LSTM")
            if cfg.batch_size // cfg.seq_len > env.num_envs * cfg.n_steps // cfg.seq_len:
                raise ValueError(f"batch_size={cfg.batch_size} asks for {cfg.batch_size // cfg.seq_len} chunks of {cfg.seq_len} steps, the "
                                 f"rollout has {env.num_envs * cfg.n_steps // cfg.seq_len}")
        if not policy.recurrent and (cfg.n_steps * env.num_envs) % min(cfg.batch_size, cfg.n_steps * env.num_envs):
            warnings.warn(f"rollout of {cfg.n_steps * env.num_envs} samples is not a multiple of batch_size={cfg.batch_size}: the last "
                          f"{(cfg.n_steps * env.num_envs) % cfg.batch_size} samples of every epoch's permutation are not trained on "
                          "(stable-baselines3 would train on them as a truncated minibatch)")
        self._fused = None
        self._fused_rec = None
        self._flat_adam = None
        fused = None
        if cfg.use_graphs and on_gpu:
            lib = native.load()
            self._flat_adam = FlatAdam(flatten_parameters(self.policy), lib, cfg.learning_rate, cfg.max_grad_norm)
            if not policy.recurrent:
                self._fused = FusedPPOStep(self.policy, lib, cfg.clip_range, cfg.ent_coef, cfg.vf_coef)
                if getattr(policy, "use_sde", False) and self._fused.merged is None:
                    self._fused = self._flat_adam = None
            elif cfg.bf16 and os.environ.get("MYO_RECURRENT_AUTOGRAD") != "1":
                self._fused_rec = FusedRecurrentPPOStep.create(self.policy, lib, cfg.clip_range, cfg.ent_coef, cfg.vf_coef)
            fused = self._fused if self._fused is not None else self._fused_rec
            if fused is not None:
                self._flat_adam.shadow = fused.half[0]
                fused.adam_syncs_shadow = True
                fused.refresh_shadow()
        self.optimizer = torch.optim.Adam(self.policy.parameters(), lr=cfg.learning_rate, eps=1e-5,
                                          capturable=on_gpu, foreach=True if on_gpu else None)
        self.world = dist.get_world_size() if dist.is_available() and dist.is_initialized() else 1
        self._hp = None
        if self._flat_adam is not None:
            self._hp = torch.zeros(HP_WORDS, device=self.device)
            self._flat_adam.hp = self._hp
            if fused is not None:
                fused.hp = self._hp
        self._current_progress_remaining = 1.0
        self._total_timesteps = None
        self._lr_now, self._clip_now = float(cfg.learning_rate), float(cfg.clip_range)
        self._hp_write()
        if self._fused is not None and self.world == 1 and os.environ.get("MYO_ADAM_SEPARATE") != "1":
            self._fused.adam = self._flat_adam
        self.rank = dist.get_rank() if self.world > 1 else 0
        N, T, O, A = env.num_envs, cfg.n_steps, env.obs_dim, env.act_dim
        d = self.device
        self.obs_buf = torch.zeros((T, N, O), device=d)
        self.act_buf = torch.zeros((T, N, A), device=d)
        self.rew_buf = torch.zeros((T, N), device=d)
        self.val_buf = torch.zeros((T, N), device=d)
        self.logp_buf = torch.zeros((T, N), device=d)
        self.start_buf = torch.zeros((T, N), device=d)
        self._last_obs = None
        self._last_starts = torch.ones(N, device=d)
        self._state = policy.initial_state(N, d)
        self._rollout_state0 = None
        self._snap_state, self._snap_full, self._snap_spare, self._snap_h, self._snap_c = None, None, None, None, None
        self.num_timesteps = 0
        self.n_updates = 0
        self.ep_returns: list = []
        self.ep_lengths: list = []
        self.gen = torch.Generator(device=self.device if on_gpu else "cpu")
        self.gen.manual_seed(seed + 1000 * self.rank)
        nparam = sum(p.numel() for p in self.policy.parameters())
        self._flat_grad = self.policy._flat["g"] if self._flat_adam is not None else torch.zeros(nparam, device=d)
        self.timers: Dict[str, float] = {"rollout": 0.0, "gae": 0.0, "update": 0.0}
        self._rollout_ready = False
        self._native = False
        self._gB2 = None
        self._sde_W = None
        self._t_host = 0
        self._last_values = None
        self.vn_allreduce_seconds, self.vn_allreduce_calls = 0.0, 0
        self._ep_log, self._ep_t, self._ep_nan_t, self.ep_info_buffer = None, 0, None, None
        self._graph, self._gs, self._graph_fb, self._graph_ap, self._graph_epoch, self._epoch_chunk = None, None, None, None, None, 0
        self._rgraph, self._rg, self._rgraph_fb, self._rgraph_ap, self._rgraph_L = None, None, None, None, None
        self._allreduce_in_graph = False
        self._early_stopped, self._last_diag = False, None

    def _autocast(self):
        on = self.cfg.bf16 and self.device.type == "cuda"
        return torch.autocast(device_type=self.device.type, dtype=torch.bfloat16, enabled=on)

    def _graphed_rollout(self) -> bool:
        return self.cfg.use_graphs and self.device.type == "cuda" and hasattr(self.env, "step_tensor")

    @torch.no_grad()
    def _rollout_policy_part(self):
        if self.cfg.seq_len is not None and self.policy.recurrent:
            L = self.cfg.seq_len
            slot = torch.where(self._t_idx % L == 0, torch.div(self._t_idx, L, rounding_mode="floor"), self._snap_spare)
            for dst, src in zip(self._snap_full, self._state_s):
                dst.index_copy_(0, slot, src.unsqueeze(0))
        with self._autocast():
            if self.policy.recurrent:
                actions, values, logp, new_state = self.policy.act(self._obs_s, self._state_s, self._starts_s)
                for dst, src in zip(self._state_new, new_state):
                    dst.copy_(src)
            else:
                actions, values, logp, _ = self.policy.act(self._obs_s, None, None)
        self._act_s.copy_(actions); self._val_s.copy_(values); self._logp_s.copy_(logp)
        self._clip_s.copy_(torch.clamp(actions, -1.0, 1.0))

    @torch.no_grad()
    def _rollout_post_part(self, raw):
        cfg = self.cfg
        outs = self._vec.process_step(*raw) if self._vec is not None else raw
        nobs, rew, done, trunc, term, comps, ep = outs
        with self._autocast():
            if self.policy.recurrent:
                tv = self.policy.predict_values(term, self._state_new, None)
            else:
                tv = self.policy.predict_values(term)
        rew = rew + cfg.gamma * tv * trunc.to(rew.dtype)
        idx = self._t_idx
        self.obs_buf.index_copy_(0, idx, self._obs_s.unsqueeze(0))
        self.act_buf.index_copy_(0, idx, self._act_s.unsqueeze(0))
        self.rew_buf.index_copy_(0, idx, rew.unsqueeze(0))
        self.val_buf.index_copy_(0, idx, self._val_s.unsqueeze(0))
        self.logp_buf.index_copy_(0, idx, self._logp_s.unsqueeze(0))
        self.start_buf.index_copy_(0, idx, self._starts_s.unsqueeze(0))
        self._obs_s.copy_(nobs)
        self._starts_s.copy_(done.to(torch.float32))
        if self.policy.recurrent:
            for dst, src in zip(self._state_s, self._state_new):
                dst.copy_(src)
# ... 474 lines not shown
            kl, cf, el = (float(x) / cnt for x in hp[HP_SUM_KL:HP_SUM_KL + 3])
            if cfg.target_kl is not None:
                if self.world == 1:
                    self.n_updates += int(hi[HP_APPLIED])
                    self._early_stopped = bool(hi[HP_STOP])
                pl, vl = hp[HP_LAST_PL], hp[HP_LAST_VL]
        else:
            kl, cf, el = (float(x) for x in torch.stack(diag).mean(0)) if diag else (float("nan"),) * 3
        y, err = ret.reshape(-1), (ret - self.val_buf).reshape(-1)
        var_y = float(y.var(unbiased=False))
        ev = float("nan") if var_y == 0 else 1.0 - float(err.var(unbiased=False)) / var_y
        stats.update(policy_loss=float(pl), value_loss=float(vl), n_updates=self.n_updates, approx_kl=kl, clip_fraction=cf,
                     entropy_loss=el, explained_variance=ev, learning_rate=self._lr_now, clip_range=self._clip_now,
                     early_stopped=self._early_stopped)
        return stats

    def _train_eager(self, adv, ret):
        cfg, pol = self.cfg, self.policy
        T, N = cfg.n_steps, self.env.num_envs
        if pol.recurrent and cfg.seq_len is not None:
            L = cfg.seq_len
            n_items, k = N * (T // L), cfg.batch_size // L
            snaps = self.rollout_snapshots()

            def evaluate(items):
                return self._chunk_loss(items, snaps, adv, ret)
        elif pol.recurrent:
            n_items, k = N, max(1, min(N, cfg.batch_size // T))

            def evaluate(idx):
                st0 = tuple(x[:, idx] for x in self._rollout_state0)
                with self._autocast():
                    v, lp, ent = pol.evaluate_actions(self.obs_buf[:, idx], self.act_buf[:, idx], st0, self.start_buf[:, idx])
                return self._loss(v.reshape(-1), lp.reshape(-1), ent, self.logp_buf[:, idx].reshape(-1),
                                  adv[:, idx].reshape(-1), ret[:, idx].reshape(-1))
        else:
            n_items = B = T * N
            k = min(cfg.batch_size, B)
            obs, act = self.obs_buf.view(B, -1), self.act_buf.view(B, -1)
            oldlp, advf, retf = self.logp_buf.view(B), adv.view(B), ret.view(B)

            def evaluate(idx):
                with self._autocast():
                    v, lp, ent = pol.evaluate_actions(obs[idx], act[idx])
                return self._loss(v, lp, ent, oldlp[idx], advf[idx], retf[idx])
        for _ in range(cfg.n_epochs):
            diag = []
            perm = torch.randperm(n_items, generator=self.gen, device=self.device)
            for s in range(0, n_items - k + 1, k):
                loss, pl, vl = evaluate(perm[s:s + k])
                diag.append(torch.stack(self._last_diag))
                if self._kl_exceeded(self._last_diag[0]):
                    self._early_stopped = True
                    break
                self.optimizer.zero_grad(set_to_none=True)
                loss.backward()
                self._allreduce_grads()
                torch.nn.utils.clip_grad_norm_(pol.parameters(), cfg.max_grad_norm)
                self.optimizer.step()
                self.n_updates += 1
            if self._early_stopped:
                break
        return pl, vl, diag

    def _chunk_loss(self, items, snaps, adv, ret):
        N, L = self.env.num_envs, self.cfg.seq_len
        s, n = torch.div(items, N, rounding_mode="floor"), items % N
        tt = (s * L).unsqueeze(0) + torch.arange(L, device=items.device).unsqueeze(1)
        sel = lambda buf: buf[tt, n]
        st0 = tuple(x[s, 0, n].unsqueeze(0) for x in snaps)
        with self._autocast():
            v, lp, ent = self.policy.evaluate_actions(sel(self.obs_buf), sel(self.act_buf), st0, sel(self.start_buf))
        return self._loss(v.reshape(-1), lp.reshape(-1), ent, sel(self.logp_buf).reshape(-1), sel(adv).reshape(-1), sel(ret).reshape(-1))

    def _mb_forward_backward(self):
        g, cfg = self._gs, self.cfg
        idx = g["idx"]
        pl, vl = self._fused.run_indexed(g["obs"], g["act"], g["oldlp"], g["adv"], g["ret"], idx)
        g["pl"], g["vl"] = pl, vl

    def _mb_apply(self):
        self._flat_adam.step(1.0 / self.world)

    def _capture_step(self, forward_backward, g, graph_allreduce=False, epoch_steps=0):
        d = self.device
        side = torch.cuda.Stream(device=d)
        snap = self._flat_adam.snapshot()
        side.wait_stream(torch.cuda.current_stream(d))
        with torch.cuda.stream(side):
            for _ in range(2):
                forward_backward()
                if self.world > 1:
                    dist.all_reduce(self._flat_grad)
                self._mb_apply()
        torch.cuda.current_stream(d).wait_stream(side)
        torch.cuda.synchronize(d)
        fb, ap, epoch, inside = torch.cuda.CUDAGraph(), None, None, False
        if graph_allreduce and dist.get_backend() != "nccl":
            warnings.warn(f"graph_allreduce needs the nccl (RCCL) backend, this process group is {dist.get_backend()!r}: "
                          "using the eager all-reduce between the two optimizer graphs")
        elif graph_allreduce:
            try:
                with torch.cuda.graph(fb, capture_error_mode="thread_local"):
                    forward_backward()
                    dist.all_reduce(self._flat_grad, op=dist.ReduceOp.SUM)
                    self._mb_apply()
            except Exception as exc:
                raise RuntimeError("capturing the RCCL gradient all-reduce inside the optimizer hipGraph failed; run without "
                                   "graph_allreduce / MYO_GRAPH_ALLREDUCE (the eager collective between two graphs)") from exc
            inside = True
        if not inside:
            with torch.cuda.graph(fb, capture_error_mode="thread_local"):
                forward_backward()
                if self.world == 1:
                    self._mb_apply()
            if self.world > 1:
                ap = torch.cuda.CUDAGraph()
                with torch.cuda.graph(ap, capture_error_mode="thread_local"):
                    self._mb_apply()
        if epoch_steps:
            bs = g["idx"].numel()
            g["perm"] = torch.zeros(epoch_steps * bs, dtype=torch.long, device=d)
            g["perm"].copy_(torch.arange(epoch_steps * bs, device=d))
            torch.cuda.synchronize(d)
            epoch = torch.cuda.CUDAGraph()
            with torch.cuda.graph(epoch, capture_error_mode="thread_local"):
                for s in range(0, epoch_steps * bs, bs):
                    g["idx"].copy_(g["perm"][s:s + bs])
                    forward_backward()
                    self._mb_apply()
        self._flat_adam.restore(snap)
        return fb, ap, epoch, inside

    def _run_captured(self, n_items, k, g, fb, ap, stats=None, epoch=None, adv_of=None):
        cfg = self.cfg
        tkl = cfg.target_kl is not None
        device_stop = tkl and self.world == 1
        stopped = False
        for _ in range(cfg.n_epochs):
            self._hp_new_epoch()
            perm = torch.randperm(n_items, generator=self.gen, device=self.device)
            if epoch is not None:
                stopped = self._replay_epoch_chunked(perm, g, k, n_items // k, epoch, fb, device_stop)
                if not device_stop:
                    self.n_updates += n_items // k
            else:
                for s in range(0, n_items - k + 1, k):
                    g["idx"].copy_(perm[s:s + k])
                    if stats is not None:
                        items = perm[s:s + k]
                        mean, std = self._global_adv_moments((adv_of(items) if adv_of is not None else g["adv"][..., items]).double())
                        stats.copy_(torch.stack([mean, std]).float())
                    fb.replay()
                    if ap is not None:
                        dist.all_reduce(self._flat_grad, op=dist.ReduceOp.SUM)
                        if tkl and self._kl_exceeded_ranks():
                            self._early_stopped = stopped = True
                            break
                        if self._dp_check:
                            self._dp_compare("gradient after the all-reduce", self._flat_grad)
                            self._dp_compare("parameters before the optimizer step", self._flat_adam.flat["p"])
                            self._dp_compare("Adam m before the optimizer step", self._flat_adam.m)
                            self._dp_compare("Adam v before the optimizer step", self._flat_adam.v)
                            self._dp_compare("Adam step counter before the optimizer step", self._flat_adam._step)
                        ap.replay()
                        if self._dp_check:
                            self._dp_compare("gradient after the optimizer step", self._flat_grad)
                            self._dp_compare("|g|^2 partial sums", self._flat_adam.sq[:64].contiguous())
                            self._dp_compare("parameters after the optimizer step", self._flat_adam.flat["p"])
                    if not device_stop:
                        self.n_updates += 1
                if device_stop and not stopped:
                    stopped = self._hp_stopped()
            if stopped:
                break

    def _replay_epoch_chunked(self, perm, g, bs, n_mb, epoch, fb, device_stop) -> bool:
        k, done, stopped = self._epoch_chunk, 0, False
        while n_mb - done >= k and not stopped:
            g["perm"].copy_(perm[done * bs:(done + k) * bs])
            epoch.replay()
            done += k
            stopped = device_stop and done < n_mb and self._hp_stopped()
        if not stopped:
            for j in range(done, n_mb):
                g["idx"].copy_(perm[j * bs:(j + 1) * bs])
                fb.replay()
            stopped = device_stop and self._hp_stopped()
        return stopped

    _dp_check = bool(os.environ.get("MYO_DP_CHECK"))

    def _dp_compare(self, what: str, x: torch.Tensor) -> None:
        cs = x.detach().contiguous().view(torch.int32).to(torch.int64).sum().reshape(1)
        lo, hi = cs.clone(), cs.clone()
        dist.all_reduce(lo, op=dist.ReduceOp.MIN); dist.all_reduce(hi, op=dist.ReduceOp.MAX)
        if int(lo[0]) != int(hi[0]) and dist.get_rank() == 0:
            print(f"MYO_DP_CHECK: {what} differs across ranks at optimizer step {self.n_updates}", flush=True)

    def _build_graphs(self, B, bs):
        d = self.device
        self._gs = {"idx": torch.zeros(bs, dtype=torch.long, device=d),
                    "obs": self.obs_buf.view(B, -1), "act": self.act_buf.view(B, -1), "oldlp": self.logp_buf.view(B),
                    "adv": torch.zeros(B, device=d), "ret": torch.zeros(B, device=d),
                    "pl": torch.zeros((), device=d), "vl": torch.zeros((), device=d)}
        self._gs["idx"].copy_(torch.arange(bs, device=d))
        n_mb = B // bs
        self._epoch_chunk = 0
        if self.world == 1 and os.environ.get("MYO_EPOCH_GRAPH") != "0" and n_mb > 1:
            self._epoch_chunk = max(1, min(n_mb, int(os.environ.get("MYO_EPOCH_GRAPH_STEPS", "64"))))
        asked = self.world > 1 and (self.cfg.graph_allreduce or os.environ.get("MYO_GRAPH_ALLREDUCE") == "1")
        self._graph_fb, self._graph_ap, self._graph_epoch, self._allreduce_in_graph = self._capture_step(
            self._mb_forward_backward, self._gs, graph_allreduce=asked, epoch_steps=self._epoch_chunk)
        self._graph = (B, bs)

    def _train_graphed(self, adv, ret):
        cfg = self.cfg
        B = cfg.n_steps * self.env.num_envs
        bs = min(cfg.batch_size, B)
        ext = (cfg.sync_adv_moments and self.world > 1) or not cfg.normalize_advantage
        if self._fused.external_adv_stats != ext:
            self._fused.external_adv_stats = ext
            self._graph = None
        if self._graph != (B, bs):
            self._build_graphs(B, bs)
            self._hp_write()
        g = self._gs
        g["adv"].copy_(adv.view(B)); g["ret"].copy_(ret.view(B))
        if not cfg.normalize_advantage:
            self._fused.stats.copy_(torch.tensor([0.0, 1.0], device=self.device))
        self._run_captured(B, bs, g, self._graph_fb, self._graph_ap,
                           stats=self._fused.stats if ext and cfg.normalize_advantage else None,
                           epoch=None if ext else self._graph_epoch)
        self._fused.refresh_shadow()
        return g["pl"], g["vl"]

    def _rec_forward_backward(self):
        g = self._rg
        idx = g["idx"]
        L = self._rgraph_L
        if self._fused_rec is not None:
            state = (g["h0"], g["c0"]) if L is None else (g["h_snap"], g["c_snap"])
            pl, vl = self._fused_rec.run_sequences(self.obs_buf, self.act_buf, self.start_buf, self.logp_buf, g["adv"], g["ret"],
                                                   *state, idx, seq_len=L)
            g["pl"], g["vl"] = pl, vl
            return
        self._flat_grad.zero_()
        if L is not None:
            loss, pl, vl = self._chunk_loss(idx, g["state0"], g["adv"], g["ret"])
            loss.backward()
            g["pl"].copy_(pl); g["vl"].copy_(vl)
            return
        st0 = tuple(x.index_select(1, idx) for x in g["state0"])
        sel = lambda buf: buf.index_select(1, idx)
        with self._autocast():
            v, lp, ent = self.policy.evaluate_actions(sel(self.obs_buf), sel(self.act_buf), st0, sel(self.start_buf))
        loss, pl, vl = self._loss(v.reshape(-1), lp.reshape(-1), ent, sel(self.logp_buf).reshape(-1),
                                  sel(g["adv"]).reshape(-1), sel(g["ret"]).reshape(-1))
        loss.backward()
        g["pl"].copy_(pl); g["vl"].copy_(vl)

    def _build_recurrent_graphs(self, T, N, m, L=None):
        d = self.device
        state = self._rollout_state0 if L is None else self.rollout_snapshots()
        if L is not None and self._fused_rec is not None:
            state = ()
        self._rg = {"idx": torch.arange(m, device=d), "state0": tuple(torch.zeros_like(x) for x in state),
                    "adv": torch.zeros((T, N), device=d), "ret": torch.zeros((T, N), device=d),
                    "pl": torch.zeros((), device=d), "vl": torch.zeros((), device=d)}
        H = self.policy.hidden
        if self._fused_rec is not None and L is None:
            self._rg["h0"], self._rg["c0"] = torch.zeros((2, N, H), device=d), torch.zeros((2, N, H), device=d)
        elif self._fused_rec is not None:
            self._rg["h_snap"], self._rg["c_snap"] = (self._snap_h, self._snap_c) if self._snap_h is not None else \
                (torch.zeros((T // L, 2, N, H), device=d, dtype=torch.bfloat16), torch.zeros((T // L, 2, N, H), device=d))
        self._rgraph_L = L
        self._rgraph_fb, self._rgraph_ap, _, _ = self._capture_step(self._rec_forward_backward, self._rg, graph_allreduce=False,
                                                                    epoch_steps=0)
        self._rgraph = (T, N, m, L)

    def _rec_stage(self, adv, ret, T, N, m, L=None):
        cfg = self.cfg
        if self._fused_rec is not None:
            ext = (cfg.sync_adv_moments and self.world > 1) or not cfg.normalize_advantage
            if self._fused_rec.external_adv_stats != ext:
                self._fused_rec.external_adv_stats = ext
                self._rgraph = None
        if self._rgraph != (T, N, m, L):
            self._build_recurrent_graphs(T, N, m, L)
            self._hp_write()
        g = self._rg
        g["adv"].copy_(adv); g["ret"].copy_(ret)
        fr = self._fused_rec
        state = self._rollout_state0 if L is None else self.rollout_snapshots()
        if fr is None or L is None:
            for dst, src in zip(g["state0"], state):
                dst.copy_(src)
        if fr is not None:
            fr.refresh_shadow()
            hp, cp, hv, cv = state
            if L is None:
                g["h0"][0].copy_(hp[0]); g["h0"][1].copy_(hv[0]); g["c0"][0].copy_(cp[0]); g["c0"][1].copy_(cv[0])
            elif g["h_snap"] is not self._snap_h:
                g["h_snap"][:, 0:1].copy_(hp); g["h_snap"][:, 1:2].copy_(hv); g["c_snap"][:, 0:1].copy_(cp); g["c_snap"][:, 1:2].copy_(cv)
            if not cfg.normalize_advantage:
                fr.stats.copy_(torch.tensor([0.0, 1.0], device=self.device))
        return g

    def _train_recurrent_graphed(self, adv, ret):
        cfg = self.cfg
        T, N, L = cfg.n_steps, self.env.num_envs, cfg.seq_len
# ... 94 lines not shown
```

Measured before the change: 1.721 million.

## Keep bf16 weight images resident, updated by Adam, and batch advantage moments per epoch

The Adam kernel now writes the bf16 packed/transposed weight images (W1p, W2, W2T, Whp, WhT, bias) directly as it updates parameters. This lets the PPO minibatch step skip the per-step prep kernel that re-converted all weights. Advantage moments for a whole epoch chunk are computed up front in one 2D-grid launch plus a merge kernel, instead of once per minibatch. The hp record path is split into a load and an apply step, and the column sums are reduced with shuffles. The cost is extra scattered stores inside Adam, plus more state that must stay consistent across graph capture and restore.

After: 1.757 million (median of 6 runs). 2.1% higher.

```diff
diff --git a/include/myobatch.h b/include/myobatch.h
--- a/include/myobatch.h
+++ b/include/myobatch.h
@@ -298,6 +298,9 @@
 int myo_ppo_mlp_sqnorm_parts(int act_dim);
 long long myo_ppo_mlp_workspace_bytes(int B, int obs_dim, int act_dim, int hidden, long long G);
 int myo_ppo_mlp_step(const myo_ppo_mlp_desc* d, void* stream);
+int myo_ppo_mlp_step_resident(const myo_ppo_mlp_desc* d, void* stream);
+int myo_ppo_mlp_images(const myo_ppo_mlp_desc* d, void* stream);
+int myo_ppo_adv_moments_epoch(const float* adv, const int64_t* idx, int B, int n_mb, float* stats, float* scratch, void* stream);
 
 typedef struct myo_ppo_mlp_rollout_desc {
   const float* obs;
@@ -328,6 +331,12 @@
 int myo_adam_apply_hp(float* p, const float* g, float* m, float* v, int n, float lr, float b1, float b2,
                       float eps, float max_norm, float grad_scale, const int* step, const float* scratch, int nparts,
                       uint16_t* p_bf16, float* hp, void* stream);
+int myo_adam_clip_step_images(float* p, const float* g, float* m, float* v, int n, float lr, float b1, float b2,
+                              float eps, float max_norm, float grad_scale, int* step, float* scratch, uint16_t* p_bf16,
+                              float* hp, const myo_ppo_mlp_desc* images, void* stream);
+int myo_adam_apply_images(float* p, const float* g, float* m, float* v, int n, float lr, float b1, float b2,
+                          float eps, float max_norm, float grad_scale, const int* step, const float* scratch, int nparts,
+                          uint16_t* p_bf16, float* hp, const myo_ppo_mlp_desc* images, void* stream);
 
 const char* myo_last_error(void);
 const char* myo_version(void);
diff --git a/myochallenge_amd/csrc/myo_ppo_mlp.h b/myochallenge_amd/csrc/myo_ppo_mlp.h
--- a/myochallenge_amd/csrc/myo_ppo_mlp.h
+++ b/myochallenge_amd/csrc/myo_ppo_mlp.h
@@ -46,25 +46,26 @@
 };
 
 #define MLP_ADV_BLOCKS 64
+__device__ __forceinline__ void mlp_adv_merge(const float* sp, int nb, int B, float* __restrict__ stats) {
+  float cn = 0.f, cm = 0.f, c2 = 0.f;
+  for (int b = 0; b < nb; ++b) {
+    const float bn = sp[3 * b], bm = sp[3 * b + 1], b2 = sp[3 * b + 2];
+    if (bn > 0.f) {
+      const float tot = cn + bn, dl = bm - cm;
+      cm += dl * (bn / tot);
+      c2 += b2 + dl * dl * (cn * bn / tot);
+      cn = tot;
+    }
+  }
+  stats[0] = cm; stats[1] = sqrtf(c2 / (B > 1 ? B - 1 : 1));
+}
 __global__ void __launch_bounds__(256) k_mlp_prep(MlpPrepArgs P) {
   if (P.adv_nb > 0 && blockIdx.x == gridDim.x - 1) {
     __shared__ float sp[3 * MLP_ADV_BLOCKS];
     const int t = threadIdx.x;
     if (t < 3 * P.adv_nb) sp[t] = P.adv_part[t];
     __syncthreads();
-    if (t == 0) {
-      float cn = 0.f, cm = 0.f, c2 = 0.f;
-      for (int b = 0; b < P.adv_nb; ++b) {
-        const float bn = sp[3 * b], bm = sp[3 * b + 1], b2 = sp[3 * b + 2];
-        if (bn > 0.f) {
-          const float tot = cn + bn, dl = bm - cm;
-          cm += dl * (bn / tot);
-          c2 += b2 + dl * dl * (cn * bn / tot);
-          cn = tot;
-        }
-      }
-      P.adv_stats[0] = cm; P.adv_stats[1] = sqrtf(c2 / (P.B > 1 ? P.B - 1 : 1));
-    }
+    if (t == 0) mlp_adv_merge(sp, P.adv_nb, P.B, P.adv_stats);
   }
   constexpr int H = MLP_H;
   const long long tid = (long long)blockIdx.x * blockDim.x + threadIdx.x, nth = (long long)gridDim.x * blockDim.x;
@@ -96,11 +97,13 @@
   }
 }
 
-__global__ void __launch_bounds__(256) k_adv_moments(const float* __restrict__ adv, const long long* __restrict__ idx, int B,
-                                                     float* __restrict__ part) {
+__global__ void __launch_bounds__(256) k_adv_moments(const float* __restrict__ adv, const long long* __restrict__ idx_all, int B,
+                                                     float* __restrict__ part_all) {
   __shared__ float red[4];
   __shared__ float s_mean;
   const int t = threadIdx.x, nb = gridDim.x;
+  const long long* __restrict__ idx = idx_all + (size_t)blockIdx.y * B;
+  float* __restrict__ part = part_all + (size_t)blockIdx.y * 3 * nb;
   const int chunk = (B + nb - 1) / nb, lo = blockIdx.x * chunk, hi = min(B, lo + chunk), n = max(hi - lo, 0);
   constexpr int PER = 4;
   float v[PER];
@@ -124,6 +127,49 @@
   __syncthreads();
   if (t == 0) { part[3 * blockIdx.x] = (float)n; part[3 * blockIdx.x + 1] = mean; part[3 * blockIdx.x + 2] = (red[0] + red[1]) + (red[2] + red[3]); }
 }
+__global__ void __launch_bounds__(256) k_adv_merge(const float* __restrict__ part_all, int nb, int B, float* __restrict__ stats) {
+  __shared__ float sp[3 * MLP_ADV_BLOCKS];
+  const int t = threadIdx.x;
+  if (t < 3 * nb) sp[t] = part_all[(size_t)blockIdx.x * 3 * nb + t];
+  __syncthreads();
+  if (t == 0) mlp_adv_merge(sp, nb, B, stats + 2 * blockIdx.x);
+}
+
+struct MlpImgTarget {
+  unsigned short *W1p, *W2, *W2T, *Whp, *WhT;
+  float* bias;
+  int off_W1[2], off_b1[2], off_W2[2], off_b2[2], off_Wh[2], off_bh[2];
+  int O, OP, A;
+};
+__device__ __forceinline__ void mlp_img_store(const MlpImgTarget& T, int i, float x) {
+  constexpr unsigned H = MLP_H;
+#pragma unroll
+  for (int net = 0; net < 2; ++net) {
+    const unsigned Ah = net == 0 ? (unsigned)T.A : 1u;
+    unsigned j = (unsigned)(i - T.off_W2[net]);
+    if (j < H * H) {
+      const unsigned short v = mlp_f2bf(x);
+      T.W2[net * H * H + j] = v;
+      T.W2T[net * H * H + (j % H) * H + j / H] = v;
+      return;
+    }
+    j = (unsigned)(i - T.off_W1[net]);
+    if (j < H * (unsigned)T.O) { const unsigned o = j / (unsigned)T.O; T.W1p[net * H * T.OP + o * T.OP + (j - o * T.O)] = mlp_f2bf(x); return; }
+    j = (unsigned)(i - T.off_Wh[net]);
+    if (j < Ah * H) {
+      const unsigned short v = mlp_f2bf(x);
+      T.Whp[net * MLP_APM * H + j] = v;
+      T.WhT[net * H * MLP_AKP + (j % H) * MLP_AKP + j / H] = v;
+      return;
+    }
+    j = (unsigned)(i - T.off_b1[net]);
+    if (j < H) { T.bias[net * H + j] = x; return; }
+    j = (unsigned)(i - T.off_b2[net]);
+    if (j < H) { T.bias[2 * H + net * H + j] = x; return; }
+    j = (unsigned)(i - T.off_bh[net]);
+    if (j < Ah) { T.bias[4 * H + net * MLP_APM + j] = x; return; }
+  }
+}
 
 template <int KSTEPS>
 __device__ __forceinline__ void mlp_load_w(myo_bf16x8 (&bw)[8][4], const unsigned short* Wg, int w_stride, int n0, int lm, int lq) {
@@ -158,7 +204,10 @@
 
 #ifdef MLP_PROF
 __device__ unsigned long long g_mlp_prof[16];
-#define MLP_STAMP(k) { __syncthreads(); if (threadIdx.x == 0 && blockIdx.x == 3 && blockIdx.y == 0) g_mlp_prof[k] = wall_clock64(); }
+#ifndef MLP_PROF_NET
+#define MLP_PROF_NET 0
+#endif
+#define MLP_STAMP(k) { __syncthreads(); if (threadIdx.x == 0 && blockIdx.x == 3 && blockIdx.y == MLP_PROF_NET) g_mlp_prof[k] = wall_clock64(); }
 extern "C" int myo_debug_mlp_prof(unsigned long long* out) { return (int)hipMemcpyFromSymbol(out, HIP_SYMBOL(g_mlp_prof), sizeof g_mlp_prof); }
 #else
 #define MLP_STAMP(k)
@@ -628,6 +677,9 @@
   __shared__ float red[4];
   const int t = threadIdx.x, A = P.A;
   if ((int)blockIdx.x < MLP_RF_BLOCKS) {
+    const bool rec = P.hp && blockIdx.x == 0;
+    MyoHpWords hw = {};
+    if (rec && t == 0) hw = myo_hp_load(P.hp);
     float sq = 0.f;
     for (long long e = (long long)blockIdx.x * 256 + t; e < P.G; e += (long long)MLP_RF_BLOCKS * 256) {
       float s = 0.f;
@@ -639,15 +691,19 @@
     for (int off = 32; off >= 1; off >>= 1) sq += __shfl_xor(sq, off, 64);
     if ((t & 63) == 0) red[t >> 6] = sq;
     float pl = 0.f, vl = 0.f, kl = 0.f, cf = 0.f, el = 0.f;
-    if (P.hp && blockIdx.x == 0 && t < 64) {
-      pl = myo_col_sum(P.part, A, P.NB, t); vl = myo_col_sum(P.part, A + 1, P.NB, t);
-      kl = myo_col_sum(P.part, 2 * A + 3, P.NB, t); cf = myo_col_sum(P.part, 2 * A + 4, P.NB, t); el = myo_col_sum(P.part, 2 * A + 5, P.NB, t);
+    if (rec && t < 64) {
+      const float* c0 = P.part + (size_t)A * P.NB; const float* c2 = P.part + (size_t)(2 * A + 3) * P.NB;
+      for (int b = t; b < P.NB; b += 64) { pl += c0[b]; vl += c0[P.NB + b]; kl += c2[b]; cf += c2[P.NB + b]; el += c2[2 * P.NB + b]; }
+      for (int off = 32; off >= 1; off >>= 1) {
+        pl += __shfl_xor(pl, off, 64); vl += __shfl_xor(vl, off, 64); kl += __shfl_xor(kl, off, 64);
+        cf += __shfl_xor(cf, off, 64); el += __shfl_xor(el, off, 64);
+      }
     }
     __syncthreads();
     if (t == 0) {
       P.sq_part[blockIdx.x] = (red[0] + red[1]) + (red[2] + red[3]);
       if (blockIdx.x == 0) {
-        const bool stopped = P.hp ? myo_hp_record(P.hp, pl, vl, kl, cf, el) : false;
+        const bool stopped = P.hp ? myo_hp_apply(P.hp, hw, pl, vl, kl, cf, el) : false;
         if (!stopped) { const int done = P.adam_step[1]; P.adam_step[0] = done; P.adam_step[1] = done + 1; }
       }
     }
diff --git a/myochallenge_amd/csrc/myobatch.hip b/myochallenge_amd/csrc/myobatch.hip
--- a/myochallenge_amd/csrc/myobatch.hip
+++ b/myochallenge_amd/csrc/myobatch.hip
@@ -637,15 +637,25 @@
     }
   }
 }
-__device__ __forceinline__ bool myo_hp_record(float* __restrict__ hp, float pl, float vl, float kl, float cf, float el) {
+struct MyoHpWords { int stop, count; float sum_kl, sum_cf, sum_el, lim; };
+__device__ __forceinline__ MyoHpWords myo_hp_load(const float* hp) {
+  const int* hi = reinterpret_cast<const int*>(hp);
+  MyoHpWords w;
+  w.stop = hi[MYO_HP_STOP]; w.count = hi[MYO_HP_COUNT];
+  w.sum_kl = hp[MYO_HP_SUM_KL]; w.sum_cf = hp[MYO_HP_SUM_CLIPFRAC]; w.sum_el = hp[MYO_HP_SUM_ENTLOSS]; w.lim = hp[MYO_HP_KL_LIMIT];
+  return w;
+}
+__device__ __forceinline__ bool myo_hp_apply(float* hp, const MyoHpWords& w, float pl, float vl, float kl, float cf, float el) {
   int* hi = reinterpret_cast<int*>(hp);
-  if (hi[MYO_HP_STOP]) return true;
-  hp[MYO_HP_SUM_KL] += kl; hp[MYO_HP_SUM_CLIPFRAC] += cf; hp[MYO_HP_SUM_ENTLOSS] += el;
-  hi[MYO_HP_COUNT] += 1;
+  if (w.stop) return true;
+  hp[MYO_HP_SUM_KL] = w.sum_kl + kl; hp[MYO_HP_SUM_CLIPFRAC] = w.sum_cf + cf; hp[MYO_HP_SUM_ENTLOSS] = w.sum_el + el;
+  hi[MYO_HP_COUNT] = w.count + 1;
   hp[MYO_HP_LAST_KL] = kl; hp[MYO_HP_LAST_PL] = pl; hp[MYO_HP_LAST_VL] = vl;
-  const float lim = hp[MYO_HP_KL_LIMIT];
-  if (lim > 0.f && kl > lim) { hi[MYO_HP_STOP] = 1; return true; }
+  if (w.lim > 0.f && kl > w.lim) { hi[MYO_HP_STOP] = 1; return true; }
   return false;
+}
+__device__ __forceinline__ bool myo_hp_record(float* hp, float pl, float vl, float kl, float cf, float el) {
+  return myo_hp_apply(hp, myo_hp_load(hp), pl, vl, kl, cf, el);
 }
 __device__ __forceinline__ float myo_col_sum(const float* __restrict__ part, int c, int NB, int lane) {
   float a = 0.f;
@@ -1514,6 +1524,8 @@
   return MYO_OK;
 }
 
+#include "myo_ppo_mlp.h"
+
 #define MYO_SQN_BLOCKS 64
 __global__ void __launch_bounds__(256) k_grad_sqnorm(const float* __restrict__ g, int n, float gs, float* __restrict__ part,
                                                      int* __restrict__ step, const float* __restrict__ hp) {
@@ -1532,7 +1544,7 @@
                                               float* __restrict__ v, int n, float lr, float b1, float b2, float eps,
                                               float max_norm, float gs, const int* __restrict__ step,
                                               const float* __restrict__ part, unsigned short* __restrict__ p_bf16, int nparts,
-                                              float* __restrict__ hp) {
+                                              float* __restrict__ hp, MlpImgTarget img) {
   if (hp) {
     if (reinterpret_cast<const int*>(hp)[MYO_HP_STOP]) return;
     lr = hp[MYO_HP_LR];
@@ -1559,18 +1571,20 @@
     const float pn = p[i] - step_size * mi / (sqrtf(vi) * inv_sqrt_bc2 + eps);
     p[i] = pn;
     if (p_bf16) p_bf16[i] = myo_f2bf(pn);
+    if (img.W1p) mlp_img_store(img, i, pn);
   }
   if (hp && blockIdx.x == 0 && threadIdx.x == 0) reinterpret_cast<int*>(hp)[MYO_HP_APPLIED] += 1;
 }
+static const MlpImgTarget kNoImages = {};
 static int adam_clip_step(float* p, const float* g, float* m, float* v, int n, float lr, float b1, float b2,
                           float eps, float max_norm, float grad_scale, int* step, float* scratch, uint16_t* p_bf16,
-                          float* hp, void* stream) {
+                          float* hp, void* stream, const MlpImgTarget& img = kNoImages) {
   if (!p || !g || !m || !v || !step || !scratch || n <= 0) return fail(MYO_E_ARG, "myo_adam_clip_step: bad arguments");
   hipStream_t st = (hipStream_t)stream;
   const int blocks = (n + 255) / 256 < 1024 ? (n + 255) / 256 : 1024;
   hipLaunchKernelGGL(k_grad_sqnorm, dim3(MYO_SQN_BLOCKS), dim3(256), 0, st, g, n, grad_scale, scratch, step, (const float*)hp);
   hipLaunchKernelGGL(k_adam, dim3(blocks), dim3(256), 0, st, p, g, m, v, n, lr, b1, b2, eps, max_norm, grad_scale, step, scratch,
-                     (unsigned short*)p_bf16, MYO_SQN_BLOCKS, hp);
+                     (unsigned short*)p_bf16, MYO_SQN_BLOCKS, hp, img);
   LAUNCH_CHECK(0)
   return MYO_OK;
 }
@@ -1586,11 +1600,11 @@
 }
 static int adam_apply(float* p, const float* g, float* m, float* v, int n, float lr, float b1, float b2,
                       float eps, float max_norm, float grad_scale, const int* step, const float* scratch, int nparts,
-                      uint16_t* p_bf16, float* hp, void* stream) {
+                      uint16_t* p_bf16, float* hp, void* stream, const MlpImgTarget& img = kNoImages) {
   if (!p || !g || !m || !v || !step || !scratch || n <= 0 || nparts <= 0) return fail(MYO_E_ARG, "myo_adam_apply: bad arguments");
   const int blocks = (n + 255) / 256 < 1024 ? (n + 255) / 256 : 1024;
   hipLaunchKernelGGL(k_adam, dim3(blocks), dim3(256), 0, (hipStream_t)stream, p, g, m, v, n, lr, b1, b2, eps, max_norm, grad_scale, step, scratch,
-                     (unsigned short*)p_bf16, nparts, hp);
+                     (unsigned short*)p_bf16, nparts, hp, img);
   LAUNCH_CHECK(0)
   return MYO_OK;
 }
@@ -1605,7 +1619,6 @@
   return adam_apply(p, g, m, v, n, lr, b1, b2, eps, max_norm, grad_scale, step, scratch, nparts, p_bf16, hp, stream);
 }
 
-#include "myo_ppo_mlp.h"
 struct MlpWs { unsigned short *W1p, *W2, *W2T, *Whp, *WhT; float* bias; unsigned short *XT, *H1T, *H2T, *dH1T, *dH2T, *dOT; float *part, *slab, *advpart; size_t bytes; };
 static MlpWs mlp_carve(unsigned char* base, int B, int OP, int A, long long G) {
   MlpWs w;
@@ -1635,31 +1648,40 @@
 extern "C" int myo_ppo_mlp_sqnorm_parts(int act_dim) {
   return MLP_RF_BLOCKS + 2 * act_dim + 3;
 }
-extern "C" int myo_ppo_mlp_step(const myo_ppo_mlp_desc* d, void* stream) {
+static MlpPrepArgs mlp_prep_args(const myo_ppo_mlp_desc* d, const MlpWs& w, int OP) {
+  MlpPrepArgs pp;
+  pp.p = d->params; pp.O = d->O; pp.OP = OP; pp.Ah[0] = d->A; pp.Ah[1] = 1;
+  for (int k = 0; k < 2; ++k) {
+    pp.off_W1[k] = d->off_W1[k]; pp.off_b1[k] = d->off_b1[k]; pp.off_W2[k] = d->off_W2[k]; pp.off_b2[k] = d->off_b2[k];
+    pp.off_Wh[k] = d->off_Wh[k]; pp.off_bh[k] = d->off_bh[k];
+  }
+  pp.adv_part = nullptr; pp.adv_stats = nullptr; pp.adv_nb = 0; pp.B = d->B;
+  pp.W1p = w.W1p; pp.W2 = w.W2; pp.W2T = w.W2T; pp.Whp = w.Whp; pp.WhT = w.WhT; pp.bias = w.bias;
+  return pp;
+}
+static int mlp_step(const myo_ppo_mlp_desc* d, void* stream, bool resident) {
+  const char* who = resident ? "myo_ppo_mlp_step_resident" : "myo_ppo_mlp_step";
   if (!d || !d->obs || !d->act || !d->oldlp || !d->adv || !d->ret || !d->idx || !d->params || !d->grads || !d->adv_stats || !d->acc ||
       !d->workspace)
-    return fail(MYO_E_ARG, "myo_ppo_mlp_step: null argument");
+    return fail(MYO_E_ARG, "%s: null argument", who);
   const int B = d->B, O = d->O, A = d->A, OP = (O + 31) / 32 * 32;
-  if (!mlp_shape_ok(B, O, A, d->hidden)) return fail(MYO_E_UNSUPPORTED, "myo_ppo_mlp_step: needs hidden = %d, obs <= %d, act <= %d, batch a multiple of %d", MLP_H, MLP_OPMAX, MLP_APM, 64 * MLP_SPLITK);
+  if (!mlp_shape_ok(B, O, A, d->hidden)) return fail(MYO_E_UNSUPPORTED, "%s: needs hidden = %d, obs <= %d, act <= %d, batch a multiple of %d", who, MLP_H, MLP_OPMAX, MLP_APM, 64 * MLP_SPLITK);
+  if (resident && d->compute_adv_stats) return fail(MYO_E_ARG, "%s: the advantage moments are the caller's (compute_adv_stats = 0)", who);
   const MlpWs w = mlp_carve((unsigned char*)d->workspace, B, OP, A, d->G);
-  if ((long long)w.bytes > d->workspace_bytes) return fail(MYO_E_ARG, "myo_ppo_mlp_step: workspace too small (%zu bytes needed)", w.bytes);
+  if ((long long)w.bytes > d->workspace_bytes) return fail(MYO_E_ARG, "%s: workspace too small (%zu bytes needed)", who, w.bytes);
   hipStream_t st = (hipStream_t)stream;
   static bool lds_set = false;
   if (!lds_set) {
     if (hipFuncSetAttribute((const void*)k_mlp_fwdbwd, hipFuncAttributeMaxDynamicSharedMemorySize, MLP_FWDBWD_LDS) != hipSuccess)
-      return fail(MYO_E_DEVICE, "myo_ppo_mlp_step: cannot reserve %d bytes of LDS", (int)MLP_FWDBWD_LDS);
+      return fail(MYO_E_DEVICE, "%s: cannot reserve %d bytes of LDS", who, (int)MLP_FWDBWD_LDS);
     lds_set = true;
   }
-  if (d->compute_adv_stats) hipLaunchKernelGGL(k_adv_moments, dim3(MLP_ADV_BLOCKS), dim3(256), 0, st, d->adv, (const long long*)d->idx, B, w.advpart);
-  MlpPrepArgs pp;
-  pp.p = d->params; pp.O = O; pp.OP = OP; pp.Ah[0] = A; pp.Ah[1] = 1;
-  for (int k = 0; k < 2; ++k) {
-    pp.off_W1[k] = d->off_W1[k]; pp.off_b1[k] = d->off_b1[k]; pp.off_W2[k] = d->off_W2[k]; pp.off_b2[k] = d->off_b2[k];
-    pp.off_Wh[k] = d->off_Wh[k]; pp.off_bh[k] = d->off_bh[k];
-  }
-  pp.adv_part = w.advpart; pp.adv_stats = d->adv_stats; pp.adv_nb = d->compute_adv_stats ? MLP_ADV_BLOCKS : 0; pp.B = B;
-  pp.W1p = w.W1p; pp.W2 = w.W2; pp.W2T = w.W2T; pp.Whp = w.Whp; pp.WhT = w.WhT; pp.bias = w.bias;
-  hipLaunchKernelGGL(k_mlp_prep, dim3(256), dim3(256), 0, st, pp);
+  if (!resident) {
+    if (d->compute_adv_stats) hipLaunchKernelGGL(k_adv_moments, dim3(MLP_ADV_BLOCKS), dim3(256), 0, st, d->adv, (const long long*)d->idx, B, w.advpart);
+    MlpPrepArgs pp = mlp_prep_args(d, w, OP);
+    pp.adv_part = w.advpart; pp.adv_stats = d->adv_stats; pp.adv_nb = d->compute_adv_stats ? MLP_ADV_BLOCKS : 0;
+    hipLaunchKernelGGL(k_mlp_prep, dim3(256), dim3(256), 0, st, pp);
+  }
   MlpArgs a;
   a.obs = d->obs; a.act = d->act; a.oldlp = d->oldlp; a.adv = d->adv; a.ret = d->ret; a.idx = (const long long*)d->idx;
   a.log_std = d->params + d->off_log_std; a.adv_stats = d->adv_stats;
@@ -1691,6 +1713,59 @@
     hipLaunchKernelGGL(k_colmajor_finish, dim3(2 * A + 3 + (d->hp ? 1 : 0)), dim3(64), 0, st, (const float*)w.part, d->acc, B / MLP_BM, A, d->ent_coef,
                        d->grads + d->off_log_std, d->grads + d->off_bh[0], d->grads + d->off_bh[1], d->hp);
   }
+  LAUNCH_CHECK(0)
+  return MYO_OK;
+}
+extern "C" int myo_ppo_mlp_step(const myo_ppo_mlp_desc* d, void* stream) { return mlp_step(d, stream, false); }
+extern "C" int myo_ppo_mlp_step_resident(const myo_ppo_mlp_desc* d, void* stream) { return mlp_step(d, stream, true); }
+static int mlp_images_ok(const myo_ppo_mlp_desc* d, const char* who, MlpWs* w) {
+  if (!d || !d->params || !d->workspace) return fail(MYO_E_ARG, "%s: null argument", who);
+  if (!mlp_shape_ok(d->B, d->O, d->A, d->hidden)) return fail(MYO_E_UNSUPPORTED, "%s: needs hidden = %d, obs <= %d, act <= %d, batch a multiple of %d", who, MLP_H, MLP_OPMAX, MLP_APM, 64 * MLP_SPLITK);
+  *w = mlp_carve((unsigned char*)d->workspace, d->B, (d->O + 31) / 32 * 32, d->A, d->G);
+  if ((long long)w->bytes > d->workspace_bytes) return fail(MYO_E_ARG, "%s: workspace too small (%zu bytes needed)", who, w->bytes);
+  return MYO_OK;
+}
+extern "C" int myo_ppo_mlp_images(const myo_ppo_mlp_desc* d, void* stream) {
+  MlpWs w;
+  if (int rc = mlp_images_ok(d, "myo_ppo_mlp_images", &w)) return rc;
+  hipLaunchKernelGGL(k_mlp_prep, dim3(256), dim3(256), 0, (hipStream_t)stream, mlp_prep_args(d, w, (d->O + 31) / 32 * 32));
+  LAUNCH_CHECK(0)
+  return MYO_OK;
+}
+static int mlp_img_target(const myo_ppo_mlp_desc* d, int n, const char* who, MlpImgTarget* T) {
+  MlpWs w;
+  if (int rc = mlp_images_ok(d, who, &w)) return rc;
+  if (d->G != n) return fail(MYO_E_ARG, "%s: the descriptor's parameter vector has %lld elements, this one %d", who, (long long)d->G, n);
+  T->W1p = w.W1p; T->W2 = w.W2; T->W2T = w.W2T; T->Whp = w.Whp; T->WhT = w.WhT; T->bias = w.bias;
+  for (int k = 0; k < 2; ++k) {
+    const int64_t off[6] = {d->off_W1[k], d->off_b1[k], d->off_W2[k], d->off_b2[k], d->off_Wh[k], d->off_bh[k]};
+    for (int q = 0; q < 6; ++q)
+      if (off[q] < 0 || off[q] >= n) return fail(MYO_E_ARG, "%s: a tensor offset lies outside the %d parameters", who, n);
+    T->off_W1[k] = (int)off[0]; T->off_b1[k] = (int)off[1]; T->off_W2[k] = (int)off[2]; T->off_b2[k] = (int)off[3];
+    T->off_Wh[k] = (int)off[4]; T->off_bh[k] = (int)off[5];
+  }
+  T->O = d->O; T->OP = (d->O + 31) / 32 * 32; T->A = d->A;
+  return MYO_OK;
+}
+extern "C" int myo_adam_clip_step_images(float* p, const float* g, float* m, float* v, int n, float lr, float b1, float b2,
+                                         float eps, float max_norm, float grad_scale, int* step, float* scratch, uint16_t* p_bf16,
+                                         float* hp, const myo_ppo_mlp_desc* images, void* stream) {
+  MlpImgTarget T;
+  if (int rc = mlp_img_target(images, n, "myo_adam_clip_step_images", &T)) return rc;
+  return adam_clip_step(p, g, m, v, n, lr, b1, b2, eps, max_norm, grad_scale, step, scratch, p_bf16, hp, stream, T);
+}
+extern "C" int myo_adam_apply_images(float* p, const float* g, float* m, float* v, int n, float lr, float b1, float b2,
+                                     float eps, float max_norm, float grad_scale, const int* step, const float* scratch, int nparts,
+                                     uint16_t* p_bf16, float* hp, const myo_ppo_mlp_desc* images, void* stream) {
+  MlpImgTarget T;
+  if (int rc = mlp_img_target(images, n, "myo_adam_apply_images", &T)) return rc;
+  return adam_apply(p, g, m, v, n, lr, b1, b2, eps, max_norm, grad_scale, step, scratch, nparts, p_bf16, hp, stream, T);
+}
+extern "C" int myo_ppo_adv_moments_epoch(const float* adv, const int64_t* idx, int B, int n_mb, float* stats, float* scratch, void* stream) {
+  if (!adv || !idx || !stats || !scratch || B <= 0 || n_mb <= 0 || n_mb > 65535) return fail(MYO_E_ARG, "myo_ppo_adv_moments_epoch: bad arguments");
+  hipStream_t st = (hipStream_t)stream;
+  hipLaunchKernelGGL(k_adv_moments, dim3(MLP_ADV_BLOCKS, n_mb), dim3(256), 0, st, adv, (const long long*)idx, B, scratch);
+  hipLaunchKernelGGL(k_adv_merge, dim3(n_mb), dim3(256), 0, st, (const float*)scratch, MLP_ADV_BLOCKS, B, stats);
   LAUNCH_CHECK(0)
   return MYO_OK;
 }
diff --git a/myochallenge_amd/native.py b/myochallenge_amd/native.py
--- a/myochallenge_amd/native.py
+++ b/myochallenge_amd/native.py
@@ -220,6 +220,11 @@
         L.myo_ppo_mlp_workspace_bytes.argtypes = [i32, i32, i32, i32, C.c_longlong]
         L.myo_ppo_mlp_step.argtypes = [C.POINTER(PpoMlpDesc), vp]
         L.myo_ppo_mlp_sqnorm_parts.argtypes = [i32]
+        L.myo_ppo_mlp_step_resident.argtypes = [C.POINTER(PpoMlpDesc), vp]
+        L.myo_ppo_mlp_images.argtypes = [C.POINTER(PpoMlpDesc), vp]
+        L.myo_ppo_adv_moments_epoch.argtypes = [vp, vp, i32, i32, vp, vp, vp]
+        L.myo_adam_clip_step_images.argtypes = L.myo_adam_clip_step_hp.argtypes[:-1] + [C.POINTER(PpoMlpDesc), vp]
+        L.myo_adam_apply_images.argtypes = L.myo_adam_apply_hp.argtypes[:-1] + [C.POINTER(PpoMlpDesc), vp]
         L.myo_ppo_mlp_rollout_workspace_bytes.restype = C.c_longlong
         L.myo_ppo_mlp_rollout_workspace_bytes.argtypes = [i32, i32, i32]
         L.myo_ppo_mlp_rollout_refresh.argtypes = [C.POINTER(PpoMlpRolloutDesc), vp]
@@ -267,6 +272,7 @@
     "myo_batch_contact_capacity", "myo_batch_sense", "myo_batch_data",
     "myo_batch_contact_items", "myo_batch_set_render_style", "myo_batch_get_render_style",
     "myo_batch_fatigue",
+    "myo_ppo_mlp_step_resident", "myo_ppo_mlp_images", "myo_ppo_adv_moments_epoch", "myo_adam_clip_step_images", "myo_adam_apply_images",
 ]
 
 ENV_PATH_SYMBOLS = [
diff --git a/myochallenge_amd/rl/fused_mlp.py b/myochallenge_amd/rl/fused_mlp.py
--- a/myochallenge_amd/rl/fused_mlp.py
+++ b/myochallenge_amd/rl/fused_mlp.py
@@ -140,6 +140,7 @@
         self.presummed = 0
         self.shadow = None
         self.hp = None
+        self.images = None
 
     @property
     def step_count(self):
@@ -152,6 +153,20 @@
         f = self.flat
         stream = torch.cuda.current_stream(f["p"].device).cuda_stream
         p = lambda t: C.c_void_p(t.data_ptr())
+        if self.images is not None:
+            sh = p(self.shadow) if self.shadow is not None else None
+            hp = p(self.hp) if self.hp is not None else None
+            if self.presummed > 0:
+                self.lib.check(self.lib.L.myo_adam_apply_images(
+                    p(f["p"]), p(f["g"]), p(self.m), p(self.v), f["p"].numel(), self.lr, self.betas[0], self.betas[1],
+                    self.eps, self.max_norm, float(grad_scale), p(self._step), p(self.sq), int(self.presummed), sh, hp,
+                    C.byref(self.images), C.c_void_p(stream)))
+            else:
+                self.lib.check(self.lib.L.myo_adam_clip_step_images(
+                    p(f["p"]), p(f["g"]), p(self.m), p(self.v), f["p"].numel(), self.lr, self.betas[0], self.betas[1],
+                    self.eps, self.max_norm, float(grad_scale), p(self._step), p(self.sq), sh, hp, C.byref(self.images),
+                    C.c_void_p(stream)))
+            return
         if self.hp is not None:
             sh = p(self.shadow) if self.shadow is not None else None
             if self.presummed > 0:
@@ -183,6 +198,9 @@
             t.copy_(s)
         if self.shadow is not None:
             self.shadow.copy_(self.flat["p"])
+        if self.images is not None:
+            stream = torch.cuda.current_stream(self.flat["p"].device).cuda_stream
+            self.lib.check(self.lib.L.myo_ppo_mlp_images(C.byref(self.images), C.c_void_p(stream)))
 
 
 class FusedPPOStep:
@@ -226,6 +244,9 @@
         self.use_mfma_step = True
         self.adam = None
         self.hp = None
+        self.resident_adam = None
+        self.adv_slot = None
+        self._moments = {}
 
     def _mfma_desc(self, B, obs_all, act_all, oldlp_all, adv_all, ret_all, idx):
         from .. import native
@@ -271,7 +292,30 @@
         if self.adam is not None and self.lib.L.myo_ppo_mlp_sqnorm_parts(self.A) <= self.adam.sq.numel():
             d.sqnorm_part, d.adam_step = self.adam.sq.data_ptr(), self.adam._step.data_ptr()
         self._mfma[key] = (d, ws)
+        if self.resident_adam is not None:
+            stream = torch.cuda.current_stream(obs_all.device).cuda_stream
+            self.lib.check(self.lib.L.myo_ppo_mlp_images(C.byref(d), C.c_void_p(stream)))
         return d
+
+    def refresh_images(self):
+        stream = torch.cuda.current_stream(self.acc.device).cuda_stream
+        for d, _ in self._mfma.values():
+            if d is not None:
+                self.lib.check(self.lib.L.myo_ppo_mlp_images(C.byref(d), C.c_void_p(stream)))
+
+    def moments_buffers(self, n_mb):
+        hit = self._moments.get(n_mb)
+        if hit is None:
+            dev = self.acc.device
+            hit = self._moments[n_mb] = (torch.zeros((n_mb, 2), device=dev), torch.zeros(192 * n_mb, device=dev))
+        return hit
+
+    def epoch_moments(self, adv_all, idx, B, n_mb):
+        hit = self.moments_buffers(n_mb)
+        stream = torch.cuda.current_stream(adv_all.device).cuda_stream
+        self.lib.check(self.lib.L.myo_ppo_adv_moments_epoch(C.c_void_p(adv_all.data_ptr()), C.c_void_p(idx.data_ptr()), B, n_mb,
+                                                            C.c_void_p(hit[0].data_ptr()), C.c_void_p(hit[1].data_ptr()), C.c_void_p(stream)))
+        return hit[0]
 
     def rollout_desc(self, obs, seed, draw, t_idx, obs_buf, act_buf, val_buf, logp_buf, clipped):
         from .. import native
@@ -316,9 +360,20 @@
         self.lib.check(self.lib.L.myo_ppo_mlp_rollout(C.byref(d), C.c_void_p(stream)))
 
     def _mfma_step(self, d):
-        d.compute_adv_stats = 0 if self.external_adv_stats else 1
         stream = torch.cuda.current_stream(self.acc.device).cuda_stream
-        self.lib.check(self.lib.L.myo_ppo_mlp_step(C.byref(d), C.c_void_p(stream)))
+        if self.resident_adam is not None:
+            slot = self.adv_slot if self.adv_slot is not None else self.stats
+            if self.adv_slot is None and not self.external_adv_stats:
+                self.lib.check(self.lib.L.myo_ppo_adv_moments_epoch(C.c_void_p(d.adv), C.c_void_p(d.idx), d.B, 1, C.c_void_p(slot.data_ptr()),
+                                                                    C.c_void_p(self.moments_buffers(1)[1].data_ptr()), C.c_void_p(stream)))
+            d.compute_adv_stats, d.adv_stats = 0, slot.data_ptr()
+            self.lib.check(self.lib.L.myo_ppo_mlp_step_resident(C.byref(d), C.c_void_p(stream)))
+            self.resident_adam.images = d
+        else:
+            d.compute_adv_stats, d.adv_stats = (0 if self.external_adv_stats else 1), self.stats.data_ptr()
+            self.lib.check(self.lib.L.myo_ppo_mlp_step(C.byref(d), C.c_void_p(stream)))
+            if self.adam is not None:
+                self.adam.images = None
         if self.adam is not None:
             self.adam.presummed = self.lib.L.myo_ppo_mlp_sqnorm_parts(self.A) if d.sqnorm_part else 0
         return self.acc[self.A], self.acc[self.A + 1]
diff --git a/myochallenge_amd/rl/ppo.py b/myochallenge_amd/rl/ppo.py
--- a/myochallenge_amd/rl/ppo.py
+++ b/myochallenge_amd/rl/ppo.py
@@ -134,6 +134,8 @@
         self._hp_write()
         if self._fused is not None and self.world == 1 and os.environ.get("MYO_ADAM_SEPARATE") != "1":
             self._fused.adam = self._flat_adam
+        if self._fused is not None and os.environ.get("MYO_PPO_RESIDENT") != "0":
+            self._fused.resident_adam = self._flat_adam
         self.rank = dist.get_rank() if self.world > 1 else 0
         N, T, O, A = env.num_envs, cfg.n_steps, env.obs_dim, env.act_dim
         d = self.device
@@ -774,7 +776,7 @@
     def _mb_apply(self):
         self._flat_adam.step(1.0 / self.world)
 
-    def _capture_step(self, forward_backward, g, graph_allreduce=False, epoch_steps=0):
+    def _capture_step(self, forward_backward, g, graph_allreduce=False, epoch_steps=0, epoch_begin=None, step_begin=None):
         d = self.device
         side = torch.cuda.Stream(device=d)
         snap = self._flat_adam.snapshot()
@@ -816,11 +818,19 @@
             g["perm"].copy_(torch.arange(epoch_steps * bs, device=d))
             torch.cuda.synchronize(d)
             epoch = torch.cuda.CUDAGraph()
-            with torch.cuda.graph(epoch, capture_error_mode="thread_local"):
-                for s in range(0, epoch_steps * bs, bs):
-                    g["idx"].copy_(g["perm"][s:s + bs])
-                    forward_backward()
-                    self._mb_apply()
+            try:
+                with torch.cuda.graph(epoch, capture_error_mode="thread_local"):
+                    if epoch_begin is not None:
+                        epoch_begin()
+                    for s in range(0, epoch_steps * bs, bs):
+                        if step_begin is not None:
+                            step_begin(s // bs)
+                        g["idx"].copy_(g["perm"][s:s + bs])
+                        forward_backward()
+                        self._mb_apply()
+            finally:
+                if step_begin is not None:
+                    step_begin(None)
         self._flat_adam.restore(snap)
         return fb, ap, epoch, inside
 
@@ -902,8 +912,19 @@
         if self.world == 1 and os.environ.get("MYO_EPOCH_GRAPH") != "0" and n_mb > 1:
             self._epoch_chunk = max(1, min(n_mb, int(os.environ.get("MYO_EPOCH_GRAPH_STEPS", "64"))))
         asked = self.world > 1 and (self.cfg.graph_allreduce or os.environ.get("MYO_GRAPH_ALLREDUCE") == "1")
+        fused, hooks = self._fused, {}
+        if fused.resident_adam is not None and self._epoch_chunk and not fused.external_adv_stats:
+            k = self._epoch_chunk
+            fused.moments_buffers(k)
+
+            def epoch_begin():
+                self._chunk_moments = fused.epoch_moments(self._gs["adv"], self._gs["perm"], bs, k)
+
+            def step_begin(j):
+                fused.adv_slot = None if j is None else self._chunk_moments[j]
+            hooks = dict(epoch_begin=epoch_begin, step_begin=step_begin)
         self._graph_fb, self._graph_ap, self._graph_epoch, self._allreduce_in_graph = self._capture_step(
-            self._mb_forward_backward, self._gs, graph_allreduce=asked, epoch_steps=self._epoch_chunk)
+            self._mb_forward_backward, self._gs, graph_allreduce=asked, epoch_steps=self._epoch_chunk, **hooks)
         self._graph = (B, bs)
 
     def _train_graphed(self, adv, ret):
@@ -919,6 +940,8 @@
             self._hp_write()
         g = self._gs
         g["adv"].copy_(adv.view(B)); g["ret"].copy_(ret.view(B))
+        if self._fused.resident_adam is not None:
+            self._fused.refresh_images()
         if not cfg.normalize_advantage:
             self._fused.stats.copy_(torch.tensor([0.0, 1.0], device=self.device))
         self._run_captured(B, bs, g, self._graph_fb, self._graph_ap,
```
